# peterpengwei/bwa-mem-quickassist

Hardware: AMD Instinct MI355X
Metric: aligned reads/sec (150 bp PE vs hg38) at 1/2/4/8 MI355X; SAM bit-exact vs CPU (higher is better)
Workload: dtype int16; 1 GPU; pe10m -- BASELINE.json configs[2]: 10000000 x 2 x 150bp read pairs per GPU per step through the whole DP path (fused seed extension with the right extension started from the device's left score, ksw_global2 + traceback, mate-rescue ksw_align2), task generator in place of the hg38 index (SURVEY.md §8d), streamed in 2 chunks, inputs resident in HBM; seeding, chaining and SAM text are host stages out; pairs_per_gpu=10000000, reads_per_gpu=20000000, chunks=2, seeded_reads_per_gpu=19999921, global_tasks_per_gpu=17000000, rescue_tasks_per_gpu=600000, rescue_batches=1, streams=3, parallelism=static shard x1, one process per GPU, no collective on the data path

## Files before the change

### bwa-mem-quickassist_amd/__init__.py

```python
import ctypes as C
import os

import numpy as np

_HERE = os.path.dirname(os.path.abspath(__file__))
LIB_PATH = os.path.join(_HERE, "libbwamem_hip.so")
DROPIN_PATH = os.path.join(_HERE, "libbwamem_hip_dropin.so")
HEADER_PATH = os.path.join(os.path.dirname(_HERE), "include", "bwamem_hip.h")

BMH_OK, BMH_E_NODEVICE, BMH_E_HIP, BMH_E_ARG, BMH_E_RANGE, BMH_E_NOMEM, BMH_E_CIGAR_CAP = 0, -1, -2, -3, -4, -5, -6
BMH_F_QREV, BMH_F_TREV, BMH_F_TPAC, BMH_F_QCOMP = 1, 2, 4, 8

EXT_TASK = np.dtype([("q_off", "<u8"), ("t_off", "<u8"), ("qlen", "<u2"), ("tlen", "<u2"),
                     ("h0", "<i4"), ("w", "<i2"), ("end_bonus", "<i2"), ("flags", "<u2"),
                     ("rsv", "<u2")])
EXT_RES = np.dtype([("score", "<i4"), ("qle", "<i4"), ("tle", "<i4"), ("gtle", "<i4"),
                    ("gscore", "<i4"), ("max_off", "<i4")])
SEED_TASK = np.dtype([("q_off", "<u8"), ("t_off", "<u8"), ("l_query", "<i4"), ("qbeg", "<i4"), ("len", "<i4"),
                      ("rbeg", "<i4"), ("wlen", "<i4"), ("flags", "<u2"), ("rsv", "<u2")])
SEED_RES = np.dtype([("qb", "<i4"), ("qe", "<i4"), ("rb", "<i4"), ("re", "<i4"), ("score", "<i4"), ("truesc", "<i4"),
                     ("w", "<i4"), ("n_ext", "<i4")])
GLB_TASK = np.dtype([("q_off", "<u8"), ("t_off", "<u8"), ("qlen", "<u2"), ("tlen", "<u2"),
                     ("w", "<i4"), ("cigar_off", "<u4"), ("cigar_cap", "<u4")])
GLB_RES = np.dtype([("score", "<i4"), ("n_cigar", "<i4")])
# ... 84 lines not shown
    _fields_ = [("l_seq", C.c_int32), ("name", C.c_char_p), ("comment", C.c_char_p), ("seq", C.c_void_p), ("qual", C.c_char_p), ("sam", C.c_void_p)]


class _RefAnn(C.Structure):
    _fields_ = [("offset", C.c_int64), ("len", C.c_int32), ("n_ambs", C.c_int32), ("gi", C.c_uint32), ("name", C.c_char_p), ("anno", C.c_char_p)]


class _RefIdx(C.Structure):
    _fields_ = [("l_pac", C.c_int64), ("n_seqs", C.c_int32), ("seed", C.c_uint32), ("anns", C.POINTER(_RefAnn))]


def make_refidx(contigs, l_pac=None, names=None):
    anns = (_RefAnn * max(len(contigs), 1))()
    for i, (off, ln) in enumerate(contigs):
        anns[i] = _RefAnn(int(off), int(ln), 0, 0, names[i] if names is not None else b"seq%d" % i, b"")
    idx = _RefIdx(int(l_pac if l_pac is not None else contigs[-1][0] + contigs[-1][1]), len(contigs), 11, anns)
    idx._keep = anns
    return idx


class _ChainStats(C.Structure):
    _fields_ = [("reads", C.c_int64), ("chains_in", C.c_int64), ("chains_out", C.c_int64), ("seeds", C.c_int64), ("equal_keys", C.c_int64),
                ("kernel_ms", C.c_float)]


CHAIN_OPT = np.dtype([("w", "<i4"), ("max_chain_gap", "<i4"), ("min_seed_len", "<i4"), ("max_occ", "<i4"), ("split_len", "<i4"),
                      ("split_width", "<i4"), ("mask_level", "<f4"), ("chain_drop_ratio", "<f4")])


def _take_chains(out, n):
    res = []
    for k in range(n):
        chains = []
        for ci in range(out[k].n):
            c = out[k].a[ci]
            sd = np.zeros(c.n, dtype=SEED)
            if c.n:
                C.memmove(sd.ctypes.data, c.seeds, c.n * SEED.itemsize)
            chains.append(sd)
            _libc.free(c.seeds)
        if out[k].a:
            _libc.free(C.cast(out[k].a, C.c_void_p))
        res.append(chains)
    return res


class _DriverStats(C.Structure):
    _fields_ = [(n, C.c_int64) for n in ("rounds", "ext_tasks", "seeds_extended", "seeds_skipped", "pool_bytes", "seeds_speculated", "short_sw")]


_lib = None


def lib():
    global _lib
    if _lib is None:
        if not os.path.exists(LIB_PATH):
            raise BmhError(BMH_E_NODEVICE, f"{LIB_PATH} not built; run __graft_entry__.build()")
        L = C.CDLL(LIB_PATH)
        L.bmh_strerror.restype = C.c_char_p
        L.bmh_last_error.restype = C.c_char_p
        L.bmh_last_error.argtypes = [C.c_void_p]
        for name in ("bmh_ctx_destroy", "bmh_ctx_sync"):
            getattr(L, name).argtypes = [C.c_void_p]
        L.bmh_ctx_create.argtypes = [C.POINTER(C.c_void_p), C.c_int]
        L.bmh_ctx_set_params.argtypes = [C.c_void_p, C.c_void_p]
        L.bmh_ctx_set_stream.argtypes = [C.c_void_p, C.c_void_p]
        L.bmh_ctx_set_qcap.argtypes = [C.c_void_p, C.c_int]
        L.bmh_ctx_set_wide_extension.argtypes = [C.c_void_p, C.c_int]
        L.bmh_extend_wide_stats.argtypes = [C.c_void_p, C.POINTER(C.c_int64), C.POINTER(C.c_float)]
        L.bmh_global_long_stats.argtypes = [C.c_void_p, C.POINTER(C.c_int64), C.POINTER(C.c_float)]
        L.bmh_ctx_set_wide_sw.argtypes = [C.c_void_p, C.c_int]
        L.bmh_sw_wide_stats.argtypes = [C.c_void_p, C.POINTER(C.c_int64), C.POINTER(C.c_float)]
        L.bmh_ctx_reserve_staging.argtypes = [C.c_void_p, C.c_size_t, C.c_size_t]
        L.bmh_ctx_reserve_device.argtypes = [C.c_void_p, C.c_size_t, C.c_int64, C.c_size_t]
        L.bmh_ctx_reserve_kernels.argtypes = [C.c_void_p, C.c_int, C.c_int, C.c_int64, C.c_int]
        L.bmh_ctx_set_pac.argtypes = [C.c_void_p, C.c_void_p, C.c_int64]
        L.bmh_set_kernel_timing.argtypes = [C.c_void_p, C.c_int]
        L.bmh_last_kernel_ms.argtypes = [C.c_void_p, C.POINTER(C.c_float)]
        L.bmh_last_extend_bin_ms.argtypes = [C.c_void_p, C.POINTER(C.c_float)]
        L.bmh_last_global_bin_ms.argtypes = [C.c_void_p, C.POINTER(C.c_float)]
        L.bmh_last_global_bands.argtypes = [C.c_void_p, C.c_void_p, C.c_int64]
        L.bmh_last_global_bin_counts.argtypes = [C.c_void_p, C.c_void_p]
        L.bmh_ctx_set_extend_rows.argtypes = [C.c_void_p, C.c_int64]
        L.bmh_last_extend_rows.argtypes = [C.c_void_p, C.c_void_p, C.c_int64]
        L.bmh_last_extend_bands.argtypes = [C.c_void_p, C.c_void_p, C.c_int64]
        L.bmh_last_seedext_round_ms.argtypes = [C.c_void_p, C.POINTER(C.c_float)]
        L.bmh_extend_bin_ms_sum.argtypes = [C.c_void_p, C.POINTER(C.c_double), C.POINTER(C.c_longlong), C.c_int]
        L.bmh_upload_pool.argtypes = [C.c_void_p, C.c_void_p, C.c_size_t]
        L.bmh_extend_batch.argtypes = [C.c_void_p, C.c_void_p, C.c_size_t, C.c_void_p, C.c_int64, C.c_void_p]
        L.bmh_extend_batch_device.argtypes = [C.c_void_p, C.c_void_p, C.c_void_p, C.c_int64, C.c_void_p, C.c_void_p]
        L.bmh_seedext_batch.argtypes = [C.c_void_p, C.c_void_p, C.c_size_t, C.c_void_p, C.c_int64, C.c_void_p]
        L.bmh_seedext_batch_device.argtypes = [C.c_void_p, C.c_void_p, C.c_void_p, C.c_int64, C.c_void_p]
        L.bmh_seedext_submit.argtypes = [C.c_void_p, C.c_void_p, C.c_int64]
        L.bmh_seedext_wait.argtypes = [C.c_void_p, C.c_void_p]
        L.bmh_seedext_stats.argtypes = [C.c_void_p, C.c_void_p]
        L.bmh_ctx_set_bwt.argtypes = [C.c_void_p, C.c_void_p]
        L.bmh_smem_batch.argtypes = [C.c_void_p, C.c_void_p, C.c_int, C.c_void_p, C.c_void_p, C.c_void_p, C.c_size_t, C.c_void_p,
                                     C.c_void_p, C.c_size_t]
        L.bmh_sa_batch.argtypes = [C.c_void_p, C.c_void_p, C.c_int64, C.c_void_p]
        L.bmh_chain_batch.argtypes = [C.c_void_p, C.c_void_p, C.c_int64, C.c_int, C.c_void_p, C.c_void_p, C.c_void_p, C.c_void_p,
                                      C.c_void_p, C.c_void_p, C.c_void_p, C.c_uint64, C.c_void_p]
        L.bmh_seed_chain_batch.argtypes = [C.c_void_p, C.c_void_p, C.c_void_p, C.c_int64, C.c_int, C.c_void_p, C.c_void_p]
        L.bmh_chain_stats.argtypes = [C.c_void_p, C.c_void_p]
        L.bmh_matesw_batch.argtypes = [C.c_void_p, C.c_int64, C.c_void_p, C.c_int, C.c_void_p, C.c_void_p, C.c_void_p,
                                       C.c_void_p, C.c_void_p, C.c_void_p, C.c_void_p]
        L.bmh_matesw_device.argtypes = [C.c_void_p, C.c_int64, C.c_int, C.c_void_p, C.c_void_p, C.c_void_p, C.c_void_p, C.c_float,
                                        C.c_void_p]
        L.bmh_sw_batch.argtypes = [C.c_void_p, C.c_void_p, C.c_size_t, C.c_void_p, C.c_int64, C.c_void_p]
        L.bmh_sw_batch_device.argtypes = [C.c_void_p, C.c_void_p, C.c_void_p, C.c_int64, C.c_void_p]
        L.bmh_extend_batch_sharded.argtypes = [C.POINTER(C.c_void_p), C.c_int, C.c_void_p, C.c_size_t, C.c_void_p,
                                               C.c_int64, C.c_void_p]
        L.bmh_global_batch.argtypes = [C.c_void_p, C.c_void_p, C.c_size_t, C.c_void_p, C.c_int64, C.c_void_p,
                                       C.c_void_p, C.c_size_t]
        L.bmh_global_batch_device.argtypes = [C.c_void_p, C.c_void_p, C.c_void_p, C.c_int64, C.c_void_p, C.c_void_p,
                                              C.c_void_p]
        L.bmh_chain2aln_batch.argtypes = [C.c_void_p, C.c_int64, C.c_void_p, C.c_int, C.c_void_p, C.c_void_p,
                                          C.c_void_p, C.c_void_p, C.c_void_p]
        L.bmh_driver_stats.argtypes = [C.c_void_p, C.c_void_p]
        L.bmh_chains2regs_batch.argtypes = [C.c_void_p, C.c_int64, C.c_void_p, C.c_int, C.c_void_p, C.c_void_p, C.c_int, C.c_void_p]
        L.bmh_chains2regs_device.argtypes = [C.c_void_p, C.c_int64, C.c_int, C.c_void_p, C.c_void_p, C.c_int, C.c_void_p]
        L.bmh_seed_chain_regs_batch.argtypes = [C.c_void_p, C.c_void_p, C.c_void_p, C.c_int64, C.c_int, C.c_void_p, C.c_int, C.c_void_p]
        L.bmh_sort_dedup_batch.argtypes = [C.c_void_p, C.c_int, C.c_void_p, C.c_float]
        L.bmh_ctx_set_regs_dedup.argtypes = [C.c_void_p, C.c_int, C.c_float]
        L.bmh_last_dedup_stats.argtypes = [C.c_void_p, C.POINTER(C.c_int64), C.POINTER(C.c_int64), C.POINTER(C.c_float)]
        L.bmh_pestat_candidates.argtypes = [C.c_void_p, C.c_int64, C.c_int, C.c_void_p, C.c_void_p]
        L.bmh_pestat_from_candidates.argtypes = [C.c_void_p, C.c_int64, C.c_void_p, C.c_void_p, C.c_int]
        L.bmh_pestat_device.argtypes = [C.c_void_p, C.c_void_p, C.c_int64, C.c_int, C.c_void_p, C.c_void_p]
        L.bmh_ctx_set_regs_drop_exact.argtypes = [C.c_void_p, C.c_int]
        L.bmh_ctx_set_pestat_collect.argtypes = [C.c_void_p, C.c_int, C.c_void_p]
        L.bmh_last_pestat_candidates.argtypes = [C.c_void_p, C.c_void_p, C.c_int64, C.POINTER(C.c_float)]
        L.bmh_last_drop_exact_stats.argtypes = [C.c_void_p, C.POINTER(C.c_int64)]
        L.bmh_decide_batch.argtypes = [C.c_void_p, C.c_int64, C.c_void_p, C.c_int64, C.c_int] + [C.c_void_p] * 6
        L.bmh_decide_device.argtypes = [C.c_void_p] + L.bmh_decide_batch.argtypes
        L.bmh_ctx_set_decide_device.argtypes = [C.c_void_p, C.c_int]
        L.bmh_last_decide_stats.argtypes = [C.c_void_p, C.POINTER(C.c_int64), C.POINTER(C.c_int64), C.POINTER(C.c_float)]
        L.bmh_wanted_cigar_batch.argtypes = [C.c_void_p, C.c_void_p, C.c_void_p, C.c_int, C.c_int] + [C.c_void_p] * 7 + [C.c_size_t, C.c_void_p, C.c_size_t]
        L.bmh_wanted_cigar_device.argtypes = L.bmh_wanted_cigar_batch.argtypes
        L.bmh_ctx_set_refidx.argtypes = [C.c_void_p, C.c_void_p]
        L.bmh_ctx_set_wanted_device.argtypes = [C.c_void_p, C.c_int]
        L.bmh_phase2_device.argtypes = ([C.c_void_p] * 5 + [C.c_int64, C.c_int] + [C.c_void_p] * 8 + [C.c_int64, C.c_void_p, C.c_void_p, C.c_size_t,
                                        C.c_void_p, C.c_size_t])
        L.bmh_ctx_set_phase2_device.argtypes = [C.c_void_p, C.c_int]
        L.bmh_last_phase2_stats.argtypes = [C.c_void_p, C.c_void_p]
        L.bmh_sam_text_batch.argtypes = [C.c_void_p, C.c_void_p, C.c_void_p, C.c_int] + [C.c_void_p] * 10 + [C.c_char_p, C.c_void_p, C.c_void_p]
        L.bmh_sam_text_device.argtypes = [C.c_void_p] + L.bmh_sam_text_batch.argtypes
        L.bmh_ctx_set_refnames.argtypes = [C.c_void_p, C.c_void_p]
        L.bmh_ctx_set_samtext_device.argtypes = [C.c_void_p, C.c_int]
        L.bmh_last_samtext_stats.argtypes = [C.c_void_p, C.c_void_p]
        L.bmh_phase2_text_device.argtypes = [C.c_void_p] * 5 + [C.c_int64, C.c_int, C.c_void_p, C.c_void_p, C.c_char_p, C.c_void_p, C.c_void_p]
        L.bmh_ctx_set_phase2_text_device.argtypes = [C.c_void_p, C.c_int]
        L.bmh_last_phase2_text_stats.argtypes = [C.c_void_p, C.c_void_p]
        L.bmh_reads_sam_device.argtypes = [C.c_void_p, C.c_void_p, C.c_void_p, C.c_int, C.c_void_p, C.c_void_p, C.c_void_p, C.c_int64, C.c_int,
                                           C.c_void_p, C.c_char_p, C.c_void_p, C.c_void_p]
        L.bmh_last_reads_sam_stats.argtypes = [C.c_void_p, C.c_void_p]
        L.bmh_last_wanted_stats.argtypes = [C.c_void_p, C.POINTER(C.c_int64), C.POINTER(C.c_int64), C.POINTER(C.c_int64), C.POINTER(C.c_float)]
        L.bmh_region_cigar_batch.argtypes = [C.c_void_p, C.c_void_p, C.c_size_t, C.c_size_t, C.c_void_p, C.c_int64, C.c_void_p, C.c_int64,
                                             C.c_size_t, C.c_int, C.c_int, C.c_void_p, C.c_void_p, C.c_void_p]
        L.bmh_region_cigar_batch.restype = C.c_int
        L.bmh_region_cigar_batch_long.argtypes = L.bmh_region_cigar_batch.argtypes + [C.POINTER(C.c_void_p), C.POINTER(C.c_int64),
                                                                                      C.POINTER(C.c_void_p), C.POINTER(C.c_void_p)]
        L.bmh_region_cigar_batch_long.restype = C.c_int
        L.bmh_last_region_long_stats.argtypes = [C.c_void_p, C.POINTER(C.c_int64), C.POINTER(C.c_int64), C.POINTER(C.c_int64), C.POINTER(C.c_float)]
        L.bmh_ctx_set_region_long.argtypes = [C.c_void_p, C.c_int]
        L.bmh_last_reg2cigar_stats.argtypes = [C.c_void_p, C.POINTER(C.c_int64), C.POINTER(C.c_int64), C.POINTER(C.c_int64)]
        L.bmh_reg2cigar_batch.argtypes = [C.c_void_p, C.c_int64, C.c_void_p, C.c_void_p, C.c_int64, C.c_void_p, C.c_void_p,
# ... 49 lines not shown
        self._check(lib().bmh_ctx_set_stream(self._h, C.c_void_p(hip_stream_ptr)))

    def set_pac(self, pac, l_pac):
        pac = np.ascontiguousarray(pac, dtype=np.uint8)
        self._pac = pac
        self._check(lib().bmh_ctx_set_pac(self._h, _ptr(pac), int(l_pac)))
        return pac

    def set_qcap(self, q):
        self._check(lib().bmh_ctx_set_qcap(self._h, int(q)))

    def set_wide_extension(self, on=True):
        self._check(lib().bmh_ctx_set_wide_extension(self._h, 1 if on else 0))

    def extend_wide_stats(self):
        n, ms = C.c_int64(0), C.c_float(-1)
        self._check(lib().bmh_extend_wide_stats(self._h, C.byref(n), C.byref(ms)))
        return int(n.value), float(ms.value)

    def global_long_stats(self):
        n, ms = C.c_int64(0), C.c_float(-1)
        self._check(lib().bmh_global_long_stats(self._h, C.byref(n), C.byref(ms)))
        return int(n.value), float(ms.value)

    def set_wide_sw(self, on=True):
        self._check(lib().bmh_ctx_set_wide_sw(self._h, 1 if on else 0))

    def sw_wide_stats(self):
        n, ms = C.c_int64(0), C.c_float(-1)
        self._check(lib().bmh_sw_wide_stats(self._h, C.byref(n), C.byref(ms)))
        return int(n.value), float(ms.value)

    def reserve_staging(self, upload_bytes, download_bytes):
        self._check(lib().bmh_ctx_reserve_staging(self._h, int(upload_bytes), int(download_bytes)))

    def reserve_device(self, pool_bytes, max_tasks, cigar_words):
        self._check(lib().bmh_ctx_reserve_device(self._h, int(pool_bytes), int(max_tasks), int(cigar_words)))

    def reserve_kernels(self, seed_reads, seed_read_len, global_tasks, global_rows):
        self._check(lib().bmh_ctx_reserve_kernels(self._h, int(seed_reads), int(seed_read_len), int(global_tasks), int(global_rows)))

    def sync(self):
        self._check(lib().bmh_ctx_sync(self._h))

    def set_kernel_timing(self, on=True):
        self._check(lib().bmh_set_kernel_timing(self._h, 1 if on else 0))

    def last_kernel_ms(self):
        ms = C.c_float(-1)
        self._check(lib().bmh_last_kernel_ms(self._h, C.byref(ms)))
        return ms.value

    def last_extend_bin_ms(self):
        ms = (C.c_float * 6)()
        self._check(lib().bmh_last_extend_bin_ms(self._h, ms))
        return [float(x) for x in ms]

    def extend_bin_ms_sum(self, reset=True):
        ms = (C.c_double * 6)()
        n = C.c_longlong(0)
        self._check(lib().bmh_extend_bin_ms_sum(self._h, ms, C.byref(n), 1 if reset else 0))
        return [float(x) for x in ms], int(n.value)

    def last_seedext_round_ms(self):
        ms = (C.c_float * 4)()
        self._check(lib().bmh_last_seedext_round_ms(self._h, ms))
        return [float(x) for x in ms]

    def last_global_bin_ms(self):
        ms = (C.c_float * 3)()
        self._check(lib().bmh_last_global_bin_ms(self._h, ms))
        return [float(x) for x in ms]

    def last_global_bands(self, n):
        bands = np.zeros(int(n), dtype=np.uint8)
        self._check(lib().bmh_last_global_bands(self._h, _ptr(bands), int(n)))
        return bands

    def last_global_bin_counts(self):
        counts = np.zeros(8, dtype=np.uint32)
        self._check(lib().bmh_last_global_bin_counts(self._h, _ptr(counts)))
        return counts

    def set_extend_rows(self, cap):
        self._check(lib().bmh_ctx_set_extend_rows(self._h, int(cap)))

    def last_extend_rows(self, n):
        rows = np.zeros(int(n), dtype=np.uint16)
        self._check(lib().bmh_last_extend_rows(self._h, _ptr(rows), int(n)))
        return rows

    def last_extend_bands(self, n):
        bands = np.zeros(int(n), dtype=np.uint8)
        self._check(lib().bmh_last_extend_bands(self._h, _ptr(bands), int(n)))
        return bands

    def upload_pool(self, pool):
        pool = np.ascontiguousarray(pool, dtype=np.uint8)
        self._check(lib().bmh_upload_pool(self._h, _ptr(pool), pool.nbytes))

    def extend_batch(self, pool, tasks):
        pool = None if pool is None else np.ascontiguousarray(pool, dtype=np.uint8)
        tasks = np.ascontiguousarray(tasks, dtype=EXT_TASK)
        res = np.zeros(len(tasks), dtype=EXT_RES)
        self._check(lib().bmh_extend_batch(self._h, _ptr(pool), _nbytes(pool), _ptr(tasks), len(tasks), _ptr(res)))
        return res

    def seedext_batch(self, pool, tasks):
        pool = None if pool is None else np.ascontiguousarray(pool, dtype=np.uint8)
        tasks = np.ascontiguousarray(tasks, dtype=SEED_TASK)
        res = np.zeros(len(tasks), dtype=SEED_RES)
        self._check(lib().bmh_seedext_batch(self._h, _ptr(pool), _nbytes(pool), _ptr(tasks), len(tasks), _ptr(res)))
        return res

    def seedext_submit(self, tasks):
        tasks = np.ascontiguousarray(tasks, dtype=SEED_TASK)
        self._check(lib().bmh_seedext_submit(self._h, _ptr(tasks), len(tasks)))
        self._seed_pending = len(tasks)

    def seedext_wait(self):
        n, self._seed_pending = getattr(self, "_seed_pending", None) or 0, None
        res = np.zeros(n, dtype=SEED_RES)
        self._check(lib().bmh_seedext_wait(self._h, _ptr(res) if n else None))
        return res

    def seedext_batch_device(self, d_pool, d_tasks, n, d_res):
        self._check(lib().bmh_seedext_batch_device(self._h, C.c_void_p(d_pool), C.c_void_p(d_tasks), int(n), C.c_void_p(d_res)))

    def seedext_stats(self):
        st = (C.c_int64 * 5)()
        self._check(lib().bmh_seedext_stats(self._h, st))
        return dict(zip(("seeds", "left_tasks", "left_retries", "right_tasks", "right_retries"), [int(x) for x in st]))

    def global_batch(self, pool, tasks, cigar_words):
        pool = None if pool is None else np.ascontiguousarray(pool, dtype=np.uint8)
        tasks = np.ascontiguousarray(tasks, dtype=GLB_TASK)
        res = np.zeros(len(tasks), dtype=GLB_RES)
        cig = np.zeros(max(int(cigar_words), 1), dtype=np.uint32)
        self._check(lib().bmh_global_batch(self._h, _ptr(pool), _nbytes(pool), _ptr(tasks), len(tasks), _ptr(res),
                                           _ptr(cig), int(cigar_words)))
        return res, cig

    def region_cigar_batch(self, readpool, opool_bytes, reqs, tasks, task_cigar_words, cig_cap=24, md_cap=64):
        readpool = np.ascontiguousarray(readpool, dtype=np.uint8)
        reqs = np.ascontiguousarray(reqs, dtype=REGION_REQ)
        tasks = np.ascontiguousarray(tasks, dtype=GLB_TASK)
        res = np.zeros(len(reqs), dtype=REGION_RES)
        cig = np.zeros((max(len(reqs), 1), cig_cap), dtype=np.uint32)
        md = np.zeros((max(len(reqs), 1), md_cap), dtype=np.uint8)
        self._check(lib().bmh_region_cigar_batch(self._h, _ptr(readpool), readpool.nbytes, int(opool_bytes), _ptr(reqs), len(reqs),
                                                 _ptr(tasks), len(tasks), int(task_cigar_words), int(cig_cap), int(md_cap), _ptr(res),
                                                 _ptr(cig), _ptr(md)))
        return res, cig, md

    def region_cigar_batch_long(self, readpool, opool_bytes, reqs, tasks, task_cigar_words, cig_cap=24, md_cap=64, guard=0):
        readpool = np.ascontiguousarray(readpool, dtype=np.uint8)
        reqs = np.ascontiguousarray(reqs, dtype=REGION_REQ)
        tasks = np.ascontiguousarray(tasks, dtype=GLB_TASK)
        n = len(reqs)
        res_b = np.full(n * REGION_RES.itemsize + guard + 1, 0x5A, dtype=np.uint8)
        cig_b = np.full(max(n, 1) * cig_cap * 4 + guard, 0x5A, dtype=np.uint8)
        md_b = np.full(max(n, 1) * md_cap + guard, 0x5A, dtype=np.uint8)
        longs, n_long, lcig, lmd = C.c_void_p(), C.c_int64(-1), C.c_void_p(), C.c_void_p()
        self._check(lib().bmh_region_cigar_batch_long(self._h, _ptr(readpool), readpool.nbytes, int(opool_bytes), _ptr(reqs), n, _ptr(tasks),
                                                      len(tasks), int(task_cigar_words), int(cig_cap), int(md_cap), _ptr(res_b), _ptr(cig_b),
                                                      _ptr(md_b), C.byref(longs), C.byref(n_long), C.byref(lcig), C.byref(lmd)))
# ... 728 lines not shown
```

### bwa-mem-quickassist_amd/csrc/api.hip

```cpp
#include <algorithm>
#include <cstdio>
#include <cstdlib>
#include <cstring>
#include <functional>
#include <mutex>
#include <new>
#include <numeric>
#include <optional>
#include <vector>

#include "bmh_ctx.h"
#include "decide.h"
#include "wanted.h"
#include "samtext.h"
#include "../host/handoff_core.h"
#include "../host/pestat_core.h"

namespace bmh {

bmh_gate_fn g_gate_enter = nullptr, g_gate_leave = nullptr;
int g_wait_blocking = 0;

int set_hip_error(bmh_ctx *ctx, hipError_t e, const char *what)
{
// ... 178 lines not shown
	case BMH_E_HIP: return "HIP runtime error";
	case BMH_E_ARG: return "invalid argument";
	case BMH_E_RANGE: return "task outside the supported range";
	case BMH_E_NOMEM: return "out of memory";
	case BMH_E_CIGAR_CAP: return "CIGAR longer than the reserved slot range";
	default: return "unknown error";
	}
}

const char *bmh_last_error(const bmh_ctx_t *ctx) { return ctx ? ctx->last_error.c_str() : "null context"; }

int bmh_device_count(int *n)
{
	int c = 0;
	if (!n) return BMH_E_ARG;
	if (hipGetDeviceCount(&c) != hipSuccess) {
		*n = 0;
		return BMH_E_NODEVICE;
	}
	*n = c;
	return BMH_OK;
}

int bmh_ctx_create(bmh_ctx_t **out, int device)
{
	if (!out) return BMH_E_ARG;
	*out = nullptr;
	int c = 0;
	if (hipGetDeviceCount(&c) != hipSuccess || c <= 0) return BMH_E_NODEVICE;
	if (device < 0 || device >= c) return BMH_E_ARG;
	bmh_ctx *ctx = new (std::nothrow) bmh_ctx();
	if (!ctx) return BMH_E_NOMEM;
	ctx->device = device;
	hipError_t e;
	if ((e = hipSetDevice(device)) == hipSuccess && g_wait_blocking) {
		if (hipSetDeviceFlags(hipDeviceScheduleBlockingSync) != hipSuccess) (void)hipGetLastError();
	}
	if (e != hipSuccess || (e = hipStreamCreateWithFlags(&ctx->own_stream, hipStreamNonBlocking)) != hipSuccess ||
	    (e = hipMalloc((void **)&ctx->d_err, 16)) != hipSuccess || (e = hipMemset(ctx->d_err, 0, 16)) != hipSuccess ||
	    (e = hipHostMalloc((void **)&ctx->h_err, sizeof(int), hipHostMallocDefault)) != hipSuccess ||
	    (e = hipEventCreate(&ctx->ev0)) != hipSuccess || (e = hipEventCreate(&ctx->ev1)) != hipSuccess ||
	    (e = hipEventCreateWithFlags(&ctx->ev_fork, hipEventDisableTiming)) != hipSuccess ||
	    (e = hipEventCreateWithFlags(&ctx->ev_join, hipEventDisableTiming)) != hipSuccess ||
	    (e = hipEventCreateWithFlags(&ctx->ev_join2, hipEventDisableTiming)) != hipSuccess ||
	    (e = hipEventCreateWithFlags(&ctx->ev_wait, hipEventDisableTiming | hipEventBlockingSync)) != hipSuccess) {
		fprintf(stderr, "[bwamem_hip] context creation failed: %s\n", hipGetErrorString(e));
		bmh_ctx_destroy(ctx);
		return BMH_E_NODEVICE;
	}
	for (int b = 0; b <= kExtBinsMax; ++b)
		if (hipEventCreate(&ctx->ev_bin[b]) != hipSuccess || hipEventCreate(&ctx->ev_bin_end[b]) != hipSuccess) {
			bmh_ctx_destroy(ctx);
			return BMH_E_NODEVICE;
		}
	for (int b = 0; b < 5; ++b)
		if (hipEventCreate(&ctx->ev_sround[b]) != hipSuccess) {
			bmh_ctx_destroy(ctx);
			return BMH_E_NODEVICE;
		}
	for (int b = 0; b < 4; ++b)
		if (hipEventCreate(&ctx->ev_gbin[b]) != hipSuccess) {
			bmh_ctx_destroy(ctx);
			return BMH_E_NODEVICE;
		}
	ctx->stream = ctx->own_stream;
	(void)hipDeviceGetAttribute(&ctx->ncu, hipDeviceAttributeMultiprocessorCount, device);
	if (ctx->ncu <= 0) ctx->ncu = 256;
	if (const char *m = getenv("BMH_EXT_PERSIST")) ctx->ext_persist = atoi(m) != 0;
	if (const char *m = getenv("BMH_EXT_SPLIT96")) ctx->ext_split96 = atoi(m) != 0;
	if (const char *m = getenv("BMH_EXT_GRID_MULT")) ctx->ext_grid_mult = atoi(m) > 0 ? atoi(m) : ctx->ext_grid_mult;
	if (const char *m = getenv("BMH_EXT_STOP")) ctx->ext_stop = atoi(m) != 0;
	if (const char *m = getenv("BMH_EXT_NARROW")) ctx->ext_narrow = atoi(m) != 0;
	if (const char *m = getenv("BMH_EXT_BANDKEY")) ctx->ext_bandkey = atoi(m) != 0;
	if (const char *m = getenv("BMH_EXT_SMALL")) ctx->small_batch = atoi(m) >= 0 ? atoi(m) : ctx->small_batch;
	if (getenv("BMH_EXT_MODE")) ctx->ext_mode_forced = true;
	if (const char *m = getenv("BMH_EXT_MODE")) ctx->force_kernel = !strcmp(m, "lds") ? 1 : !strcmp(m, "reg") ? 2 : !strcmp(m, "grp") ? 3 : !strcmp(m, "lanex4") ? 4 : !strcmp(m, "wide") ? 5 : 0;
	if (const char *m = getenv("BMH_GLB_MODE")) ctx->glb_mode = !strcmp(m, "wave") ? 1 : 0;
	if (const char *m = getenv("BMH_SW_MODE")) ctx->sw_mode = !strcmp(m, "generic") ? 1 : 0;
	if (const char *m = getenv("BMH_SW_WAVE")) ctx->sw_wave = atoi(m) != 0;
	if (const char *m = getenv("BMH_GL_FAST")) ctx->glb_fast = atoi(m) != 0;
	if (const char *m = getenv("BMH_GLB_C32")) ctx->glb_c32 = atoi(m) != 0;
	if (const char *m = getenv("BMH_GLB_NARROW")) ctx->glb_narrow = atoi(m) != 0;
	if (const char *m = getenv("BMH_GLB_EXACT")) ctx->glb_exact = atoi(m) >= 7 ? 7 : atoi(m) >= 3 ? 3 : 0;
	if (const char *m = getenv("BMH_GRID_MULT")) ctx->grid_mult = atoi(m) > 0 ? atoi(m) : 1;
	if (const char *m = getenv("BMH_EXT_SCHED")) ctx->ext_sched = atoi(m) >= 0 && atoi(m) <= 4 ? atoi(m) : -1;
	*out = ctx;
	return BMH_OK;
}

static void pac_release(bmh_ctx_t *ctx);
void free_bwt_binding(void *p);

int bmh_ctx_destroy(bmh_ctx_t *ctx)
{
	if (!ctx) return BMH_OK;
	(void)hipSetDevice(ctx->device);
	if (ctx->stream) (void)stream_wait(ctx, ctx->stream);
	free_buf(ctx->d_pool), free_buf(ctx->d_tasks), free_buf(ctx->d_res), free_buf(ctx->d_order);
	free_buf(ctx->d_cigar), free_buf(ctx->d_scratch), free_buf(ctx->d_bins), free_buf(ctx->d_gband), free_buf(ctx->d_ext_rows), free_buf(ctx->d_eband), free_buf(ctx->d_zslab), free_buf(ctx->d_sw), free_buf(ctx->d_swrm);
	free_buf(ctx->d_seedws), free_buf(ctx->d_region), free_buf(ctx->d_chain), free_buf(ctx->d_wide_slab), free_buf(ctx->d_c2r);
	if (ctx->d_wide_stat) (void)hipFree(ctx->d_wide_stat);
	if (ctx->d_swl_stat) (void)hipFree(ctx->d_swl_stat);
	free_buf(ctx->d_swl), free_buf(ctx->d_dedup), free_buf(ctx->d_msw), free_buf(ctx->d_decide), free_buf(ctx->d_logk);
	free(ctx->h_logk);
	free_buf(ctx->d_refidx), free_buf(ctx->d_wanted);
	if (ctx->h_wstat) (void)hipHostFree(ctx->h_wstat);
	free_buf(ctx->d_refnames), free_buf(ctx->d_samtext), free_buf(ctx->d_sam_out);
	if (ctx->h_ststat) (void)hipHostFree(ctx->h_ststat);
	if (ctx->h_ptstat) (void)hipHostFree(ctx->h_ptstat);
	for (auto &e : ctx->ev_gather)
		if (e) (void)hipEventDestroy(e);
	for (auto &e : ctx->ev_samtext)
		if (e) (void)hipEventDestroy(e);
	for (auto &e : ctx->ev_wanted)
		if (e) (void)hipEventDestroy(e);
	for (auto &e : ctx->ev_decide)
		if (e) (void)hipEventDestroy(e);
	for (auto &e : ctx->ev_chain)
		if (e) (void)hipEventDestroy(e);
	for (auto &e : ctx->ev_dedup)
		if (e) (void)hipEventDestroy(e);
	free_buf(ctx->d_rlong), free_buf(ctx->d_lcig), free_buf(ctx->d_lmd);
	for (auto &e : ctx->ev_rlong)
		if (e) (void)hipEventDestroy(e);
	free_buf(ctx->d_pestat);
	for (auto &e : ctx->ev_pestat)
		if (e) (void)hipEventDestroy(e);
	for (auto &e : ctx->ev_plan)
		if (e) (void)hipEventDestroy(e);
	for (auto &h : ctx->hint) {
		if (h.ev) (void)hipEventDestroy(h.ev);
		if (h.h) (void)hipHostFree(h.h);
	}
	pac_release(ctx);
	if (ctx->bwt_bind) free_bwt_binding(ctx->bwt_bind);
	if (ctx->d_err) (void)hipFree(ctx->d_err);
	if (ctx->h_err) (void)hipHostFree(ctx->h_err);
	if (ctx->h_up.p) (void)hipHostFree(ctx->h_up.p);
	if (ctx->h_down.p) (void)hipHostFree(ctx->h_down.p);
	if (ctx->ev0) (void)hipEventDestroy(ctx->ev0);
	if (ctx->ev1) (void)hipEventDestroy(ctx->ev1);
	for (int b = 0; b <= kExtBinsMax; ++b)
	{
		if (ctx->ev_bin[b]) (void)hipEventDestroy(ctx->ev_bin[b]);
		if (ctx->ev_bin_end[b]) (void)hipEventDestroy(ctx->ev_bin_end[b]);
	}
	for (int b = 0; b < 4; ++b)
		if (ctx->ev_gbin[b]) (void)hipEventDestroy(ctx->ev_gbin[b]);
	for (int b = 0; b < 2; ++b)
		if (ctx->ev_glong[b]) (void)hipEventDestroy(ctx->ev_glong[b]);
	for (int b = 0; b < 2; ++b)
		if (ctx->ev_swl[b]) (void)hipEventDestroy(ctx->ev_swl[b]);
	for (int b = 0; b < 5; ++b)
		if (ctx->ev_sround[b]) (void)hipEventDestroy(ctx->ev_sround[b]);
	if (ctx->ev_fork) (void)hipEventDestroy(ctx->ev_fork);
	if (ctx->ev_join) (void)hipEventDestroy(ctx->ev_join);
	if (ctx->aux_stream) (void)hipStreamDestroy(ctx->aux_stream);
	if (ctx->ev_join2) (void)hipEventDestroy(ctx->ev_join2);
	if (ctx->ev_wait) (void)hipEventDestroy(ctx->ev_wait);
	if (ctx->aux2_stream) (void)hipStreamDestroy(ctx->aux2_stream);
	if (ctx->own_stream) (void)hipStreamDestroy(ctx->own_stream);
	delete ctx;
	return BMH_OK;
}

int bmh_ctx_set_params(bmh_ctx_t *ctx, const bmh_params_t *p)
{
	if (!ctx || !p) return BMH_E_ARG;
	if (p->e_del < 0 || p->e_ins < 0 || p->o_ins < 0 || p->o_del < 0) {
		ctx->last_error = "need e_del>=0, e_ins>=0, o_del>=0, o_ins>=0";
		return BMH_E_RANGE;
	}
	ctx->params = *p;
	DevParams &d = ctx->dev;
	d.o_del = p->o_del, d.e_del = p->e_del, d.o_ins = p->o_ins, d.e_ins = p->e_ins, d.zdrop = p->zdrop;
	d.max_mat = 0;
	int mn = 0;
	for (int i = 0; i < 25; ++i) d.max_mat = std::max(d.max_mat, (int)p->mat[i]), mn = std::min(mn, (int)p->mat[i]);
	d.bias = -mn;
	{
		int8_t lo = 127;
		for (int i = 0; i < 25; ++i) lo = std::min(lo, p->mat[i]);
// ... 150 lines not shown
int bmh_ctx_sync(bmh_ctx_t *ctx)
{
	if (!ctx) return BMH_E_ARG;
	BMH_HIP(ctx, hipSetDevice(ctx->device));
	BMH_HIP(ctx, stream_wait(ctx, ctx->stream));
	return fetch_err(ctx);
}

int bmh_set_kernel_timing(bmh_ctx_t *ctx, int enable)
{
	if (!ctx) return BMH_E_ARG;
	ctx->timing = enable != 0;
	ctx->ev_valid = false;
	return BMH_OK;
}

int bmh_last_kernel_ms(bmh_ctx_t *ctx, float *ms)
{
	if (!ctx || !ms) return BMH_E_ARG;
	*ms = -1.f;
	if (!ctx->ev_valid) return BMH_OK;
	BMH_HIP(ctx, hipEventSynchronize(ctx->ev1));
	BMH_HIP(ctx, hipEventElapsedTime(ms, ctx->ev0, ctx->ev1));
	return BMH_OK;
}

int bmh_last_extend_bin_ms(bmh_ctx_t *ctx, float ms[6])
{
	if (!ctx || !ms) return BMH_E_ARG;
	for (int b = 0; b < kExtBins; ++b) ms[b] = -1.f;
	if (!ctx->ev_bin_valid) return BMH_OK;
	BMH_HIP(ctx, hipEventSynchronize(ctx->ev1));
	for (int b = 0; b < kExtBins; ++b) BMH_HIP(ctx, hipEventElapsedTime(&ms[b], ctx->ev_bin[b], ctx->ev_bin_end[b]));
	return BMH_OK;
}

int bmh_extend_bin_ms_sum(bmh_ctx_t *ctx, double ms[6], long long *launches, int reset)
{
	if (!ctx || !ms) return BMH_E_ARG;
	for (int b = 0; b < kExtBins; ++b) ms[b] = ctx->ext_bin_ms_sum[b];
	if (launches) *launches = ctx->ext_bin_launches;
	if (reset) {
		for (int b = 0; b < kExtBins; ++b) ctx->ext_bin_ms_sum[b] = 0.0;
		ctx->ext_bin_launches = 0;
	}
	return BMH_OK;
}

int bmh_last_seedext_round_ms(bmh_ctx_t *ctx, float ms[4])
{
	if (!ctx || !ms) return BMH_E_ARG;
	ms[0] = ms[1] = ms[2] = ms[3] = -1.f;
	if (!ctx->ev_sround_valid) return BMH_OK;
	BMH_HIP(ctx, hipEventSynchronize(ctx->ev_sround[4]));
	for (int b = 0; b < 4; ++b) BMH_HIP(ctx, hipEventElapsedTime(&ms[b], ctx->ev_sround[b], ctx->ev_sround[b + 1]));
	return BMH_OK;
}

int bmh_last_global_bin_ms(bmh_ctx_t *ctx, float ms[3])
{
	if (!ctx || !ms) return BMH_E_ARG;
	ms[0] = ms[1] = ms[2] = -1.f;
	if (!ctx->ev_gbin_valid) return BMH_OK;
	BMH_HIP(ctx, hipEventSynchronize(ctx->ev_gbin[3]));
	for (int b = 0; b < 3; ++b) BMH_HIP(ctx, hipEventElapsedTime(&ms[b], ctx->ev_gbin[b], ctx->ev_gbin[b + 1]));
	return BMH_OK;
}

int bmh_last_global_bands(bmh_ctx_t *ctx, uint8_t *bands, int64_t n)
{
	if (!ctx || !bands || n <= 0 || n != ctx->gband_n || !ctx->d_gband.p) return BMH_E_ARG;
	BMH_HIP(ctx, hipSetDevice(ctx->device));
	BMH_HIP(ctx, stream_wait(ctx, ctx->stream));
	BMH_HIP(ctx, hipMemcpy(bands, ctx->d_gband.p, (size_t)n, hipMemcpyDeviceToHost));
	return BMH_OK;
}

int bmh_last_global_bin_counts(bmh_ctx_t *ctx, uint32_t counts[8])
{
	if (!ctx || !counts || !ctx->gbins_valid || !ctx->d_bins.p) return BMH_E_ARG;
	BMH_HIP(ctx, hipSetDevice(ctx->device));
	BMH_HIP(ctx, stream_wait(ctx, ctx->stream));
	BMH_HIP(ctx, hipMemcpy(counts, ctx->d_bins.p, kSortBins * sizeof(uint32_t), hipMemcpyDeviceToHost));
	return BMH_OK;
}

int bmh_ctx_set_extend_rows(bmh_ctx_t *ctx, int64_t cap)
{
	if (!ctx || cap < 0 || cap > 0xffffffffLL) return BMH_E_ARG;
	ctx->ext_rows_cap = cap, ctx->ext_rows_n = 0;
	return BMH_OK;
}

int bmh_last_extend_rows(bmh_ctx_t *ctx, uint16_t *rows, int64_t n)
{
	if (!ctx || !rows || n <= 0 || n > ctx->ext_rows_n || !ctx->d_ext_rows.p) return BMH_E_ARG;
	BMH_HIP(ctx, hipSetDevice(ctx->device));
	BMH_HIP(ctx, stream_wait(ctx, ctx->stream));
	BMH_HIP(ctx, hipMemcpy(rows, ctx->d_ext_rows.p, (size_t)n * sizeof(uint16_t), hipMemcpyDeviceToHost));
	return BMH_OK;
}

int bmh_last_extend_bands(bmh_ctx_t *ctx, uint8_t *bands, int64_t n)
{
	if (!ctx || !bands || n <= 0 || n != ctx->eband_n || !ctx->d_eband.p) return BMH_E_ARG;
	BMH_HIP(ctx, hipSetDevice(ctx->device));
	BMH_HIP(ctx, stream_wait(ctx, ctx->stream));
	BMH_HIP(ctx, hipMemcpy(bands, ctx->d_eband.p, (size_t)n, hipMemcpyDeviceToHost));
	return BMH_OK;
}


int bmh_extend_batch_device(bmh_ctx_t *ctx, const uint8_t *d_pool, const bmh_ext_task_t *d_tasks, int64_t n,
                            bmh_ext_result_t *d_res, const uint32_t *d_order)
{
	if (!ctx || n < 0 || (n > 0 && (!d_pool || !d_tasks || !d_res))) return BMH_E_ARG;
	if (!ctx->have_params) return BMH_E_ARG;
	if (n > 0xffffffffLL) return BMH_E_ARG;
	BMH_HIP(ctx, hipSetDevice(ctx->device));
	return launch_extend(ctx, d_pool, d_tasks, n, d_res, d_order, ctx->qcap);
}

static int validate_ext(bmh_ctx *ctx, const bmh_ext_task_t *t, int64_t n, size_t pool_bytes, int *qmax)
{
	int qm = 1;
	for (int64_t k = 0; k < n; ++k) {
		const bmh_ext_task_t &x = t[k];
		const bool qr = x.flags & BMH_F_QREV, tr = x.flags & BMH_F_TREV, tp = x.flags & BMH_F_TPAC;
		const uint64_t qlo = qr ? x.q_off - (x.qlen ? x.qlen - 1 : 0) : x.q_off, thi_len = x.tlen;
		const uint64_t tlo = tr ? x.t_off - (x.tlen ? x.tlen - 1 : 0) : x.t_off;
		const uint64_t tspace = tp ? (uint64_t)(ctx->dev.l_pac << 1) : (uint64_t)pool_bytes;
		if (tp && !ctx->dev.pac) {
			ctx->last_error = "task " + std::to_string(k) + " has BMH_F_TPAC but no reference was uploaded (bmh_ctx_set_pac)";
			return BMH_E_ARG;
		}
		if ((qr && x.qlen && x.q_off + 1 < x.qlen) || (tr && x.tlen && x.t_off + 1 < x.tlen) || qlo + x.qlen > pool_bytes ||
		    tlo + thi_len > tspace) {
			ctx->last_error = "task " + std::to_string(k) + " reads outside the sequence pool";
			return BMH_E_ARG;
		}
		const int h0 = x.h0 < 0 ? 0 : x.h0;
		if (!ctx->wide_ext && (int64_t)h0 + (int64_t)x.qlen * ctx->dev.max_mat > kScoreLimit) {
			ctx->last_error = "task " + std::to_string(k) + ": h0 + qlen*max(mat) exceeds the 16-bit score range";
			return BMH_E_RANGE;
		}
		if (ctx->wide_ext && (int64_t)h0 + (int64_t)x.qlen * ctx->dev.max_mat > kWideScoreLimit) {
			ctx->last_error = "task " + std::to_string(k) + ": h0 + qlen*max(mat) exceeds the wide extension's score range (2^24)";
			return BMH_E_RANGE;
		}
		qm = std::max(qm, (int)x.qlen);
	}
	*qmax = qm;
	return BMH_OK;
}

int bmh_extend_batch(bmh_ctx_t *ctx, const uint8_t *pool, size_t pool_bytes, const bmh_ext_task_t *tasks, int64_t n,
                     bmh_ext_result_t *results)
{
	if (!ctx || n < 0 || (n > 0 && (!tasks || !results))) return BMH_E_ARG;
	if (!ctx->have_params) return BMH_E_ARG;
	if (n == 0) return BMH_OK;
	if (n > 0xffffffffLL) return BMH_E_ARG;
	if (!pool && !ctx->pool_resident) return BMH_E_ARG;
	int qmax = 1, rc;
	if ((rc = validate_ext(ctx, tasks, n, pool ? pool_bytes : ctx->pool_bytes, &qmax))) return rc;
	GateGuard gate;
// ... 618 lines not shown
	if (n > 0 && (!pool || !tasks || !results)) return BMH_E_ARG;
	std::vector<int> qmax((size_t)std::max(n_ctx, 0));
	return run_sharded(
	    ctxs, n_ctx, n,
	    [&](bmh_ctx *c, size_t g, int64_t lo, int64_t m) { return m > 0x7fffffffLL ? BMH_E_ARG : validate_seeds(c, tasks + lo, m, pool_bytes, &qmax[g]); },
	    [&](Stager &st, size_t g, int64_t lo, int64_t m) {
		    return enqueue_batch(st, false, pool, pool_bytes, tasks + lo, m, results + lo, [&](bmh_ctx *c, auto p, auto t, auto r) {
			    return launch_seedext(c, p, t, m, r, qmax[g]);
		    });
	    });
}

int bmh_sw_batch_sharded(bmh_ctx_t *const *ctxs, int n_ctx, const uint8_t *pool, size_t pool_bytes, const bmh_sw_task_t *tasks, int64_t n,
                         bmh_sw_result_t *results)
{
	if (n > 0 && (!pool || !tasks || !results)) return BMH_E_ARG;
	struct SwShape {
		int qmax = 1, tmax = 1, qmin = 65535;
	};
	std::vector<SwShape> shape((size_t)std::max(n_ctx, 0));
	return run_sharded(
	    ctxs, n_ctx, n,
	    [&](bmh_ctx *c, size_t g, int64_t lo, int64_t m) {
		    SwShape &s = shape[g];
		    return validate_sw(c, tasks + lo, m, pool_bytes, &s.qmax, &s.tmax, &s.qmin);
	    },
	    [&](Stager &st, size_t g, int64_t lo, int64_t m) {
		    return enqueue_batch(st, false, pool, pool_bytes, tasks + lo, m, results + lo, [&](bmh_ctx *c, auto p, auto t, auto r) {
			    return launch_sw(c, p, t, m, r, shape[g].qmax, shape[g].tmax, shape[g].qmin);
		    });
	    });
}

int bmh_global_batch_sharded(bmh_ctx_t *const *ctxs, int n_ctx, const uint8_t *pool, size_t pool_bytes, const bmh_glb_task_t *tasks, int64_t n,
                             bmh_glb_result_t *results, uint32_t *cigar_pool, size_t cigar_words)
{
	if (n > 0 && (!pool || !tasks || !results)) return BMH_E_ARG;
	std::vector<std::vector<uint32_t>> back((size_t)std::max(n_ctx, 0));
	std::vector<GlbShape> shape((size_t)std::max(n_ctx, 0));
	const int rc = run_sharded(
	    ctxs, n_ctx, n,
	    [&](bmh_ctx *c, size_t g, int64_t lo, int64_t m) {
		    return m > 0xffffffffLL ? BMH_E_ARG : validate_glb(c, tasks + lo, m, pool_bytes, cigar_pool != nullptr, cigar_words, &shape[g]);
	    },
	    [&](Stager &st, size_t g, int64_t lo, int64_t m) {
		    const GlbShape &gs = shape[g];
		    back[g].resize(gs.cig_hi > gs.cig_lo ? gs.cig_hi - gs.cig_lo : 0);
		    const CigarDown cig{cigar_words, back[g].data(), gs.cig_lo, back[g].size()};
		    return enqueue_batch(
		        st, false, pool, pool_bytes, tasks + lo, m, results + lo,
		        [&](bmh_ctx *c, auto p, auto t, auto r) { return launch_global(c, p, t, m, r, (uint32_t *)c->d_cigar.p, nullptr, gs.qmax, gs.tmax, gs.wmax, gs.wraw, &gs.lg); },
		        &cig);
	    });
	if (rc && rc != BMH_E_CIGAR_CAP && rc != BMH_E_RANGE) return rc;
	for (int g = 0; g < n_ctx && n > 0; ++g) {
		const int64_t lo = n * g / n_ctx, hi = n * (g + 1) / n_ctx;
		if (back[(size_t)g].empty()) continue;
		for (int64_t k = lo; k < hi; ++k) {
			const bmh_glb_task_t &x = tasks[k];
			const size_t nw = std::min<size_t>((size_t)std::max(results[k].n_cigar, 0), x.cigar_cap);
			if (nw) memcpy(cigar_pool + x.cigar_off, back[(size_t)g].data() + ((size_t)x.cigar_off - shape[(size_t)g].cig_lo), nw * 4);
		}
	}
	return rc;
}

int bmh_ctx_reserve_staging(bmh_ctx_t *ctx, size_t upload_bytes, size_t download_bytes)
{
	if (!ctx) return BMH_E_ARG;
	int rc;
	BMH_HIP(ctx, hipSetDevice(ctx->device));
	if ((rc = ensure_host(ctx, ctx->h_up, upload_bytes)) || (rc = ensure_host(ctx, ctx->h_down, download_bytes))) return rc;
	return BMH_OK;
}

int bmh_ctx_reserve_device(bmh_ctx_t *ctx, size_t pool_bytes, int64_t max_tasks, size_t cigar_words)
{
	if (!ctx || max_tasks < 0) return BMH_E_ARG;
	int rc;
	const size_t N = (size_t)max_tasks;
	BMH_HIP(ctx, hipSetDevice(ctx->device));
	if (ctx->glb_narrow && (1 + (size_t)kSortBins) * N + 16 > ctx->d_gband.cap) ctx->gband_n = 0;
	if ((16 + (size_t)kSortBins * kSortKeysHost + (N + 1) / 2 + 1 + (size_t)kSortBins * N) * 4 > ctx->d_bins.cap) ctx->gbins_valid = false;
	if ((rc = ensure(ctx, ctx->d_pool, pool_bytes + 16)) || (rc = ensure(ctx, ctx->d_tasks, N * 40 + 64)) || (rc = ensure(ctx, ctx->d_res, N * 32 + 64)) ||
	    (rc = ensure(ctx, ctx->d_cigar, (cigar_words + 4) * 4)) ||
	    (rc = ensure(ctx, ctx->d_bins, (16 + (size_t)kSortBins * kSortKeysHost + (N + 1) / 2 + 1 + (size_t)kSortBins * N) * 4)) ||
	    (ctx->glb_narrow && (rc = ensure(ctx, ctx->d_gband, (1 + (size_t)kSortBins) * N + 16))))
		return rc;
	return BMH_OK;
}

int bmh_ctx_reserve_kernels(bmh_ctx_t *ctx, int seed_reads, int seed_read_len, int64_t global_tasks, int global_rows)
{
	if (!ctx || seed_reads < 0 || seed_read_len < 0 || global_tasks < 0 || global_rows < 0) return BMH_E_ARG;
	int rc;
	BMH_HIP(ctx, hipSetDevice(ctx->device));
	if (seed_reads > 0) {
		const size_t grid = std::min<size_t>(((size_t)seed_reads + 63) / 64, 1024 * 4);
		if ((rc = ensure(ctx, ctx->d_sw, grid * 3 * ((size_t)seed_read_len + 2) * 64 * 32))) return rc;
	}
	if (global_tasks > 0) {
		const size_t grid = std::min<size_t>(((size_t)global_tasks + 63) / 64, (size_t)std::max(ctx->ncu, 1) * 4 * 2);
		if ((rc = ensure(ctx, ctx->d_zslab, grid * (size_t)std::min(global_rows, 512) * 8 * 256))) return rc;
	}
	return BMH_OK;
}


int bmh_sort_dedup_batch(bmh_ctx_t *ctx, int n_reads, bmh_alnreg_v *regs, float mask_level_redun)
{
	if (!ctx || n_reads < 0 || (n_reads > 0 && !regs)) return BMH_E_ARG;
	size_t total = 0;
	for (int r = 0; r < n_reads; ++r) {
		if (regs[r].n && !regs[r].a) return BMH_E_ARG;
		if (regs[r].n > 0x7fffffffu - total) {
			ctx->last_error = "bmh_sort_dedup_batch: more than 2^31-1 regions in the batch";
			return BMH_E_ARG;
		}
		total += regs[r].n;
	}
	if (total == 0) {
		ctx->dedup_in = ctx->dedup_out = 0, ctx->dedup_ms = -1.f;
		return BMH_OK;
	}
	const size_t nr = (size_t)n_reads, o_off = 64, o_cnt = o_off + (nr + 1) * 8, o_reg = (o_cnt + nr * 8 + 63) & ~(size_t)63;
	const size_t b_reg = total * sizeof(bmh_alnreg_t), b_up = o_reg + b_reg, b_down = b_up - o_cnt;
	std::vector<uint8_t> up, down;
	try {
		up.resize(b_up), down.resize(b_down);
	} catch (const std::bad_alloc &) {
		ctx->last_error = "bmh_sort_dedup_batch: out of host memory";
		return BMH_E_NOMEM;
	}
	memset(up.data(), 0, o_off);
	unsigned long long *off = (unsigned long long *)(up.data() + o_off), *cnt = (unsigned long long *)(up.data() + o_cnt);
	size_t at = 0;
	for (int r = 0; r < n_reads; ++r) {
		off[r] = at, cnt[r] = regs[r].n;
		if (regs[r].n) memcpy(up.data() + o_reg + at * sizeof(bmh_alnreg_t), regs[r].a, regs[r].n * sizeof(bmh_alnreg_t));
		at += regs[r].n;
	}
	off[n_reads] = at;
	memset(up.data() + o_cnt + nr * 8, 0, o_reg - (o_cnt + nr * 8));
	GateGuard gate;
	BMH_HIP(ctx, hipSetDevice(ctx->device));
	Stager st(ctx);
	unsigned long long removed = 0;
	int rc = [&]() -> int {
		int e;
		if ((e = ensure(ctx, ctx->d_dedup, b_up)) || (e = st.stage(b_up, b_down + 64))) return e;
		uint8_t *d = (uint8_t *)ctx->d_dedup.p;
		if ((e = st.h2d(d, up.data(), b_up))) return e;
		if ((e = launch_region_dedup(ctx, (bmh_alnreg_t *)(d + o_reg), (const unsigned long long *)(d + o_off), (unsigned long long *)(d + o_cnt), n_reads,
		                             (unsigned long long)total, mask_level_redun, (unsigned long long *)d, ctx->d_err)))
			return e;
		if ((e = st.d2h(down.data(), d + o_cnt, b_down)) || (e = st.d2h(&removed, d, 8))) return e;
		return BMH_OK;
	}();
	if ((rc = st.end(rc))) return rc;
	const unsigned long long *kept = (const unsigned long long *)down.data();
	const uint8_t *ra = down.data() + (o_reg - o_cnt);
	for (int r = 0; r < n_reads; ++r) {
		if (regs[r].n <= 1) continue;
		if (kept[r] > regs[r].n) {
			ctx->last_error = "bmh_sort_dedup_batch: the device's counts are inconsistent";
			return BMH_E_ARG;
// ... 1622 lines not shown
```

### bwa-mem-quickassist_amd/csrc/bmh_ctx.h

```cpp
#pragma once
#include <hip/hip_runtime.h>
#include <stdint.h>
#include <string>
#include <vector>

#include "../../include/bwamem_hip.h"
#include "bmh_device.h"
#include "../host/regplan_core.h"

constexpr int kExtBinsMax = 6;

struct DevBuf {
	void *p = nullptr;
	size_t cap = 0;
};

struct bmh_ctx {
	int device = 0;
	hipStream_t own_stream = nullptr, stream = nullptr;
	bool have_params = false;
	bool glb_params = false;
	bmh_params_t params{};
	bmh::DevParams dev{};
	int qcap = 512;
	DevBuf d_pool, d_tasks, d_res, d_order, d_cigar, d_scratch;
	void *bwt_bind = nullptr;
	double smem_calls_per_base = 0.06, smem_intv_per_base = 0.35, smem_pos_per_base = 0.03;
	const uint8_t *h_pac = nullptr;
	DevBuf d_swrm;
	DevBuf d_sw;
	DevBuf d_zslab;
	int glb_mode = 0;
	int sw_mode = 0;
	int glb_fast = 1;
	int glb_narrow = 1;
	int glb_c32 = 1;
	int glb_exact = 7;
	bool gbins_valid = false;
	DevBuf d_gband;
	int64_t gband_n = 0;
	int sw_wave = 1;
	DevBuf d_bins;
	int grid_mult = 1;
	int ext_sched = -1;
	bool ext_mode_forced = false;
	int small_batch = 49152;
	int force_kernel = 0;
	bool pool_resident = false;
	size_t pool_bytes = 0;
	DevBuf h_up, h_down;
	int *d_err = nullptr;
	int *h_err = nullptr;
	bool timing = false;
	hipEvent_t ev0 = nullptr, ev1 = nullptr;
	bool ev_valid = false;
	hipEvent_t ev_bin[kExtBinsMax + 1] = {};
	hipEvent_t ev_bin_end[kExtBinsMax + 1] = {};
	hipStream_t aux_stream = nullptr;
	hipEvent_t ev_fork = nullptr, ev_join = nullptr;
	hipStream_t aux2_stream = nullptr;
	hipEvent_t ev_join2 = nullptr;
	hipEvent_t ev_wait = nullptr;
	bool ev_bin_valid = false;
	int ext_split96 = 1;
	double ext_bin_ms_sum[kExtBinsMax + 1] = {};
	long long ext_bin_launches = 0;
	hipEvent_t ev_gbin[4] = {};
	bool ev_gbin_valid = false;
	hipEvent_t ev_sround[5] = {};
	bool ev_sround_valid = false;
	std::string last_error;
	bmh_driver_stats_t dstats{};
	int ncu = 256;
	bool ext_persist = false;
	int ext_grid_mult = 2;
	int ext_stop = 1;
	int64_t ext_rows_cap = 0;
	DevBuf d_ext_rows;
	int64_t ext_rows_n = 0;
	int ext_narrow = 1;
	int ext_bandkey = 1;
	DevBuf d_eband;
	int64_t eband_n = 0;
	static constexpr int kHintKinds = 6;
	struct BinHint {
		uint32_t *h = nullptr;
		hipEvent_t ev = nullptr;
		bool pending = false, valid = false;
		uint32_t cnt[8] = {};
	} hint[kHintKinds];
	DevBuf d_seedws;
	DevBuf d_region;
	DevBuf d_rlong;
	DevBuf d_lcig, d_lmd;
	hipEvent_t ev_rlong[4] = {};
	long long rlong_regions = -1, rlong_words = -1, rlong_md = -1;
	float rlong_ms = -1.f;
	bool region_long = false;
	long long r2c_regions = -1, r2c_long_device = -1, r2c_redone_host = -1;
	bmh_seedext_stats_t sstats{};
	int64_t seed_pending_n = -1;
	DevBuf d_chain;
	hipEvent_t ev_chain[2] = {};
	bmh_chain_stats_t cstats{-1, -1, -1, -1, -1, -1.f};
	DevBuf d_c2r;
	bool wide_ext = false;
	bool wide_last = false;
	unsigned long long *d_wide_stat = nullptr;
	double wide_ms_sum = 0.0;
	long long wide_total = 0;
	DevBuf d_wide_slab;
	hipEvent_t ev_glong[2] = {};
	double glong_ms_sum = 0.0;
	bool wide_sw = false;
	unsigned long long *d_swl_stat = nullptr;
	DevBuf d_swl;
	hipEvent_t ev_swl[2] = {};
	double swl_ms_sum = 0.0;
	bool regs_dedup = false;
	float regs_dedup_mask = 0.95f;
// ... 61 lines not shown
	{
		if (leave) leave();
	}
	GateGuard(const GateGuard &) = delete;
	GateGuard &operator=(const GateGuard &) = delete;
};

int set_hip_error(bmh_ctx *ctx, hipError_t e, const char *what);

struct DevSeedTables {
	int n_reads;
	const int *len;
	const uint32_t *coff;
	const bmh_smem_call_t *calls;
	const uint64_t *ioff;
	const bmh_smem_intv_t *intv;
	const uint64_t *sa_off, *sa_pos;
	uint64_t n_calls, n_intv, n_pos;
	const uint8_t *pool;
	const uint64_t *read_off;
};
struct DevChains {
	int n_reads;
	const unsigned long long *coff, *soff;
	const uint32_t *cn;
	const bmh_seed_t *seeds;
	const uint32_t *n_keys;
	unsigned long long tc, ts;
	unsigned long long n_equal;
	float kernel_ms;
};
int chain_compact_device(bmh_ctx *ctx, const bmh_chain_opt_t *o, int64_t l_pac, const DevSeedTables &t, DevChains *out);
typedef int (*SeedTablesFn)(bmh_ctx *ctx, const DevSeedTables &t, void *user);
int seed_tables_device(bmh_ctx *ctx, const bmh_smem_opt_t *o, int max_occ, int n_reads, const bmh_read_t *reads, SeedTablesFn fn, void *user);
struct ResidentRegs {
	const unsigned long long *roff = nullptr;
	const bmh_alnreg_t *reg = nullptr;
	long long total = 0, kmax = 1, opool_cap = 0;
	bool neg = false;
};
int reads_regs_check(bmh_ctx *ctx, const bmh_smem_opt_t *so, const bmh_chain_opt_t *co, int64_t l_pac, int n_reads, const bmh_read_t *reads,
                     int min_seed_len, const char *who);
int reads_regs_resident(bmh_ctx *ctx, const bmh_smem_opt_t *so, const bmh_chain_opt_t *co, int64_t l_pac, int n_reads, const bmh_read_t *reads,
                        int min_seed_len, const bmh_sam_opt_t *o, ResidentRegs *out);
extern int g_wait_blocking;
inline hipError_t stream_wait(bmh_ctx *ctx, hipStream_t s)
{
	if (!g_wait_blocking || !ctx->ev_wait) return hipStreamSynchronize(s);
	const hipError_t e = hipEventRecord(ctx->ev_wait, s);
	return e != hipSuccess ? e : hipEventSynchronize(ctx->ev_wait);
}
int ensure(bmh_ctx *ctx, DevBuf &b, size_t bytes);
int ensure_host(bmh_ctx *ctx, DevBuf &b, size_t bytes);

#define BMH_HIP(ctx, call)                                                   \
	do {                                                                     \
		hipError_t e_ = (call);                                              \
		if (e_ != hipSuccess) return bmh::set_hip_error((ctx), e_, #call);   \
	} while (0)

constexpr long long kPersistentGrid = 256LL * 32 * 4;

inline bool ext_gaps_too_large(const bmh_params_t &p)
{
	return (long long)p.o_del + p.e_del > 65535 || (long long)p.o_ins + p.e_ins > 65535 || p.e_del > 16383 || p.e_ins > 16383;
}
int launch_extend(bmh_ctx *ctx, const uint8_t *d_pool, const bmh_ext_task_t *d_tasks, int64_t n,
                  bmh_ext_result_t *d_res, const uint32_t *d_order, int qmax, const uint32_t *d_n = nullptr, int kind = 0);
int launch_seedext(bmh_ctx *ctx, const uint8_t *d_pool, const bmh_seed_task_t *d_tasks, int64_t n,
                   bmh_seed_result_t *d_res, int qmax);
const uint32_t *seedext_counters(const bmh_ctx *ctx);
inline long long ext_resident_waves(const bmh_ctx *ctx, int waves_per_simd) { return (long long)ctx->ncu * 4 * waves_per_simd; }
constexpr int kLdsQcap = 13632;
constexpr int kWideLdsQcap = 12544;
int launch_extend_wide(bmh_ctx *ctx, const uint8_t *d_pool, const bmh_ext_task_t *d_tasks, int64_t n, bmh_ext_result_t *d_res,
                       const uint32_t *d_order, const uint32_t *d_count, int qmax, long long grid_cap = 0);
int wide_stats_begin(bmh_ctx *ctx);
int launch_extend_lds(bmh_ctx *ctx, const uint8_t *d_pool, const bmh_ext_task_t *d_tasks, int64_t n,
                      bmh_ext_result_t *d_res, const uint32_t *d_order, const uint32_t *d_count, int qmax, long long grid_cap = 0);
constexpr int kSortKeysHost = 2048;
int sort_tasks_begin(bmh_ctx *ctx, int64_t n, uint32_t **counts, uint32_t **lists);
int sort_tasks_finish(bmh_ctx *ctx, int64_t n, const uint32_t *d_order, unsigned blocks, const uint32_t *d_n = nullptr,
                      uint32_t *d_total = nullptr, const uint8_t *d_payload = nullptr, uint8_t *d_plists = nullptr);
int launch_global_lane(bmh_ctx *ctx, int c, const uint8_t *d_pool, const bmh_glb_task_t *d_tasks, int64_t n,
                       bmh_glb_result_t *d_res, uint32_t *d_cigar, const uint32_t *d_order, const uint32_t *d_count,
                       int rows_cap, const uint8_t *d_band = nullptr);
int launch_global_narrow(bmh_ctx *ctx, int wlo, const uint8_t *d_pool, const bmh_glb_task_t *d_tasks, int64_t n, bmh_glb_result_t *d_res,
                         uint32_t *d_cigar, const uint32_t *d_order, const uint32_t *d_count, int rows_cap, const uint8_t *d_band = nullptr);
constexpr int kExtBins = 6;
constexpr int kWideBin = 6;
constexpr int kSortBins = 8;
constexpr int kGrpTcapHost = 1024;

constexpr int kCapBin = 7;
constexpr int kSortBlocks = 512;
constexpr uint16_t kNoTask = 0xffff;
static_assert(kSortBins * kSortKeysHost <= kNoTask, "binkey is 16 bits wide and keeps one value for entries without a task");

__device__ __forceinline__ int ext_bin_of(int qlen, int tlen, int mode)
{
	if (mode == 1 || qlen < 1) return 5;
	if (mode == 3 && qlen <= 256 && tlen > kGrpTcapHost) return 3;
	return qlen <= 32 ? 0 : qlen <= 64 ? 1 : qlen <= 128 ? 2 : qlen <= 256 ? 3 : (qlen <= 512 && mode == 4) ? 4 : 5;
}

__device__ __forceinline__ bool ext_goes_wide(int qlen, int h0, int max_mat)
{
	return (long long)max(h0, 0) + (long long)qlen * max_mat > kScoreLimit || qlen > kLdsQcap;
}

__device__ __forceinline__ int ext_sort_key(int bin, int qlen, int tlen, int h0, int cls = -1)
{
	if (bin > 4) return 0;
	const int qlo = bin == 0 ? 1 : (16 << bin) + 1, qsh = bin < 2 ? 1 : bin;
	const int rows = min(tlen, 2 * qlen + 8) >> (bin > 2 ? bin - 2 : 0);
	return ((max(qlen - qlo, 0) >> qsh) * 8 + (cls >= 0 ? cls : min(max(h0, 0) >> 4, 7))) * 16 + min(rows >> 4, 15);
}

struct ExtBinRule {
	int mode;
	int wide;
	int max_mat, qmax;
	bmh_ext_result_t *out;
	int *err_flag;
};

__device__ __forceinline__ int ext_task_bin(const ExtBinRule &r, int qlen, int tlen, int h0)
{
	return qlen > r.qmax ? kCapBin : r.wide && (r.wide == 2 || ext_goes_wide(qlen, h0, r.max_mat)) ? kWideBin : ext_bin_of(qlen, tlen, r.mode);
}

__device__ __forceinline__ int ext_binkey_of(const ExtBinRule &r, int qlen, int tlen, int h0, size_t idx, int cls = -1)
{
	const int bin = ext_task_bin(r, qlen, tlen, h0);
	if (bin == kCapBin) {
		int *p = (int *)(r.out + idx);
		p[0] = INT32_MIN, p[1] = p[2] = p[3] = p[4] = p[5] = 0;
		atomicExch(r.err_flag, BMH_E_RANGE);
	}
	return bin * kSortKeysHost + ext_sort_key(bin, qlen, tlen, h0, cls);
}

struct ExtBinned {
	ExtBinRule rule;
	uint32_t *hist;
	uint16_t *binkey;
	unsigned blocks;
	uint8_t *band;
	bool tiny;
};
int extend_binned_begin(bmh_ctx *ctx, int64_t n, bmh_ext_result_t *d_res, int qmax, int kind, ExtBinned *p);
int extend_binned_finish(bmh_ctx *ctx, const uint8_t *d_pool, const bmh_ext_task_t *d_tasks, int64_t n, bmh_ext_result_t *d_res,
                         int qmax, int kind, const ExtBinned &p, uint32_t *d_total);

int launch_extend_grp(bmh_ctx *ctx, int nv, const uint8_t *d_pool, const bmh_ext_task_t *d_tasks, int64_t n,
                      bmh_ext_result_t *d_res, const uint32_t *d_order, const uint32_t *d_count);
int launch_extend_lanex(bmh_ctx *ctx, int lpt, const uint8_t *d_pool, const bmh_ext_task_t *d_tasks, int64_t n,
                        bmh_ext_result_t *d_res, const uint32_t *d_order, const uint32_t *d_count, int min_count);
int launch_sw(bmh_ctx *ctx, const uint8_t *d_pool, const bmh_sw_task_t *d_tasks, int64_t n, bmh_sw_result_t *d_res,
              int qcap, int tcap, int qmin);
inline bool sw_byte_gaps_wrap(const bmh_params_t &p) { return p.o_del + p.e_del > 255 || p.o_ins + p.e_ins > 255; }
int launch_sw_lane(bmh_ctx *ctx, int b, bool corr, bool word, const uint8_t *d_pool, const bmh_sw_task_t *d_tasks, int64_t n,
                   bmh_sw_result_t *d_res, const uint32_t *d_order, const uint32_t *d_count, uint16_t *d_rm, int rows_cap,
                   int grid, int pass2, uint32_t *d_next);
bool sw_wave_fits(int64_t n, int qcap, int tcap);
int launch_sw_wave(bmh_ctx *ctx, const uint8_t *d_pool, const bmh_sw_task_t *d_tasks, int64_t n, bmh_sw_result_t *d_res, int max_cols,
                   int tcap, const uint32_t *d_order = nullptr, const uint32_t *d_count = nullptr);
int launch_sw_generic(bmh_ctx *ctx, const uint8_t *d_pool, const bmh_sw_task_t *d_tasks, int64_t n,
                      bmh_sw_result_t *d_res, const uint32_t *d_order, const uint32_t *d_count, int qcap, int tcap, int wave_cols = 0,
// ... 71 lines not shown
```

### bwa-mem-quickassist_amd/csrc/bmh_device.h

```cpp
#pragma once
#include <hip/hip_runtime.h>
#include <stdint.h>

#include "../../include/bwamem_hip.h"

namespace bmh {

struct DevParams {
	int o_del, e_del, o_ins, e_ins, zdrop;
	int max_mat;
	int bias;
	int sw_shift;
	uint32_t matw[7];
	const uint8_t *pac;
	long long l_pac;
};

constexpr int kScoreLimit = 32000;
constexpr int kWideScoreLimit = 1 << 24;
constexpr int kNegInf16 = -16384;
constexpr int kGlbLaneWorst = 12000;

constexpr int DPP_ROW_SHR1 = 0x111, DPP_ROW_SHR2 = 0x112, DPP_ROW_SHR4 = 0x114, DPP_ROW_SHR8 = 0x118;
constexpr int DPP_WAVE_SHR1 = 0x138, DPP_ROW_BCAST15 = 0x142, DPP_ROW_BCAST31 = 0x143;

template <int CTRL, int ROW_MASK = 0xf>
__device__ __forceinline__ int dpp(int old, int src)
{
	return __builtin_amdgcn_update_dpp(old, src, CTRL, ROW_MASK, 0xf, false);
}

__device__ __forceinline__ int wave_scan_max(int v)
{
	constexpr int I = INT32_MIN;
	v = max(dpp<DPP_ROW_SHR1>(I, v), v);
	v = max(dpp<DPP_ROW_SHR2>(I, v), v);
	v = max(dpp<DPP_ROW_SHR4>(I, v), v);
	v = max(dpp<DPP_ROW_SHR8>(I, v), v);
	v = max(dpp<DPP_ROW_BCAST15, 0xa>(I, v), v);
	v = max(dpp<DPP_ROW_BCAST31, 0xc>(I, v), v);
	return v;
}

__device__ __forceinline__ int wave_reduce_max(int v)
{
	return __builtin_amdgcn_readlane(wave_scan_max(v), 63);
}

__device__ __forceinline__ int wave_shr1(int v, int lane0)
{
	return dpp<DPP_WAVE_SHR1>(lane0, v);
}

__device__ __forceinline__ int uni(int v) { return __builtin_amdgcn_readfirstlane(v); }

__device__ __forceinline__ int mat_at(const DevParams &P, int idx)
{
	return (int)(int8_t)(P.matw[idx >> 2] >> ((idx & 3) * 8));
}

__device__ __forceinline__ int seq_base(const uint8_t *pool, uint64_t off, int k, bool rev)
{
	return rev ? pool[off - (uint64_t)k] : pool[off + (uint64_t)k];
}

__device__ __forceinline__ int tgt_base(const uint8_t *pool, const DevParams &P, uint64_t off, int k, bool rev, bool tpac)
{
	if (!tpac) return seq_base(pool, off, k, rev);
	const long long p = rev ? (long long)off - k : (long long)off + k;
	const bool rs = p >= P.l_pac;
	const long long f = rs ? (P.l_pac << 1) - 1 - p : p;
	const int b = P.pac[f >> 2] >> ((~f & 3) << 1) & 3;
	return rs ? 3 - b : b;
}

#define BMH_OP16(name, text)                                                                                            \
	__device__ __forceinline__ int name(int a, int b)                                                                   \
	{                                                                                                                   \
		int d;                                                                                                          \
		asm(text " %0, %1, %2" : "=v"(d) : "v"(a), "v"(b));                                                             \
		return d;                                                                                                       \
	}
BMH_OP16(add16, "v_add_u16")
BMH_OP16(sub16, "v_sub_u16")
BMH_OP16(max16, "v_max_i16")
#undef BMH_OP16
__device__ __forceinline__ int maxu16(int a, int b)
{
	int d;
	asm("v_max_u16 %0, %1, %2" : "=v"(d) : "v"(a), "v"(b));
	return d;
}
__device__ __forceinline__ int subc16(int a, int k)
{
	int d;
	asm("v_sub_u16_e64 %0, %1, %2 clamp" : "=v"(d) : "v"(a), "s"(k));
	return d;
}
__device__ __forceinline__ int nonzero16(int a)
{
	int d;
	asm("v_min_u16 %0, 1, %1" : "=v"(d) : "v"(a));
	return d;
}
__device__ __forceinline__ int subk16(int a, int k)
{
	int d;
	asm("v_subrev_u16 %0, %1, %2" : "=v"(d) : "s"(k), "v"(a));
	return d;
}
template <int B> __device__ __forceinline__ int add_score(int sc4, int r)
{
	int d;
	if constexpr (B == 0) asm("v_add_u32_sdwa %0, sext(%1), %2 dst_sel:DWORD dst_unused:UNUSED_PAD src0_sel:BYTE_0 src1_sel:WORD_0" : "=v"(d) : "v"(sc4), "v"(r));
	if constexpr (B == 1) asm("v_add_u32_sdwa %0, sext(%1), %2 dst_sel:DWORD dst_unused:UNUSED_PAD src0_sel:BYTE_1 src1_sel:WORD_0" : "=v"(d) : "v"(sc4), "v"(r));
	if constexpr (B == 2) asm("v_add_u32_sdwa %0, sext(%1), %2 dst_sel:DWORD dst_unused:UNUSED_PAD src0_sel:BYTE_2 src1_sel:WORD_0" : "=v"(d) : "v"(sc4), "v"(r));
	if constexpr (B == 3) asm("v_add_u32_sdwa %0, sext(%1), %2 dst_sel:DWORD dst_unused:UNUSED_PAD src0_sel:BYTE_3 src1_sel:WORD_0" : "=v"(d) : "v"(sc4), "v"(r));
	return d;
}
__device__ __forceinline__ void max16_into_hi(int &r, int a, int b)
{
	asm("v_max_i16_sdwa %0, %1, %2 dst_sel:WORD_1 dst_unused:UNUSED_PRESERVE src0_sel:WORD_0 src1_sel:WORD_0" : "+v"(r) : "v"(a), "v"(b));
}

__device__ __forceinline__ void sub16_into_hi(int &r, int a, int b)
{
	asm("v_sub_u16_sdwa %0, %1, %2 dst_sel:WORD_1 dst_unused:UNUSED_PRESERVE src0_sel:WORD_0 src1_sel:WORD_0" : "+v"(r) : "v"(a), "v"(b));
}

__device__ __forceinline__ int band_cap(int qlen, int mx, int end_bonus, int o, int e)
{
	int x = qlen * mx + end_bonus - o;
	return x >= 0 ? x / e + 1 : 1;
}

}
```

### bwa-mem-quickassist_amd/csrc/global_kernel.hip

```cpp
#include "bmh_ctx.h"
#include "bmh_device.h"
#include "../host/glbband_core.h"
#include "../host/glbbin_core.h"

namespace bmh {

constexpr int kNegInf = -0x40000000;

struct CigarSink {
	uint32_t *base;
	int cap, nw, last_op, last_len;
	__device__ __forceinline__ void flush(int lane)
	{
		if (last_len > 0) {
			if (nw < cap && lane == 0) base[cap - 1 - nw] = (uint32_t)last_len << 4 | (uint32_t)last_op;
			++nw;
		}
	}
	__device__ __forceinline__ void push(int op, int len, int lane)
	{
		if (len <= 0) return;
		if (last_len > 0 && op == last_op) last_len += len;
		else {
			flush(lane);
// ... 187 lines not shown
				}
			}
			if (n_cigar > cigar_cap && lane == 0) atomicExch(err_flag, BMH_E_CIGAR_CAP);
		}
		if (lane == 0) out[idx].score = score, out[idx].n_cigar = n_cigar;
	}
}

__device__ __forceinline__ bool glb_lane_domain(const DevParams &P, int qlen, int tlen, int w, int lane_ok, int rows_cap)
{
	const int emax = max(P.e_del, P.e_ins), smax = max(P.bias, P.max_mat);
	const int worst = P.o_del + P.o_ins + emax * (qlen + tlen) + smax * max(qlen, tlen);
	return lane_ok && tlen <= rows_cap && worst < kGlbLaneWorst && P.o_del + P.o_ins < 4000 && w >= 0;
}

constexpr int kBandThreads = 256, kBandLanes = 8;
__global__ __launch_bounds__(kBandThreads) void glb_band_kernel(const uint8_t *__restrict__ pool, const bmh_glb_task_t *__restrict__ tasks,
                                                                const uint32_t *__restrict__ order, long long n, uint8_t *__restrict__ band,
                                                                DevParams P, int lane_ok, int rows_cap)
{
	__shared__ int8_t smat[32];
	if (threadIdx.x < 25) smat[threadIdx.x] = (int8_t)mat_at(P, threadIdx.x);
	__syncthreads();
	const int amax = bmh_glbband_amax(smat);
	const bool rule = bmh_glbband_applies(amax, P.o_del, P.e_del, P.o_ins, P.e_ins);
	const int g = threadIdx.x & (kBandLanes - 1);
	constexpr int kPer = kBandThreads / kBandLanes;
	for (long long k = (long long)blockIdx.x * kPer + threadIdx.x / kBandLanes; k < n; k += (long long)gridDim.x * kPer) {
		const uint32_t idx = order ? order[k] : (uint32_t)k;
		const uint4 *tp = (const uint4 *)(tasks + idx);
		const uint4 ta = tp[0], tb = tp[1];
		const int qlen = (int)(tb.x & 0xffff), tlen = (int)(tb.x >> 16);
		int w = (int)tb.y;
		if (rule && qlen >= 1 && tlen >= 1 && w >= abs(qlen - tlen) && glb_lane_domain(P, qlen, tlen, w, lane_ok, rows_cap)) {
			const bmh_gb_walk_t wk = bmh_glbband_walk(P.o_del, P.e_del, P.o_ins, P.e_ins, pool + ((uint64_t)ta.y << 32 | ta.x), qlen,
			                                          pool + ((uint64_t)ta.w << 32 | ta.z), tlen);
			const int per = ((wk.n + 8 * kBandLanes - 1) / (8 * kBandLanes)) * 8;
			const int from = min(g * per, wk.n), to = min(from + per, wk.n);
			const bmh_gb_part_t mine = bmh_glbband_part(smat, &wk, from, to);
			bmh_gb_part_t acc = {0, 0, 0};
#pragma unroll
			for (int j = 0; j < kBandLanes; ++j) {
				const bmh_gb_part_t nx = {__shfl(mine.s1, j, kBandLanes), __shfl(mine.d, j, kBandLanes), __shfl(mine.b, j, kBandLanes)};
				bmh_glbband_join(&acc, &nx);
			}
			w = bmh_glbband_from_lb(amax, P.o_del, P.e_del, P.o_ins, P.e_ins, qlen, tlen, w, acc.s1 + acc.b - wk.gap);
		}
		if (g == 0) band[k] = (uint8_t)(w < 0 || w > 255 ? 255 : w);
	}
}

__global__ __launch_bounds__(256) void glb_sort_hist_kernel(const bmh_glb_task_t *__restrict__ tasks,
                                                            const uint32_t *__restrict__ order, long long n,
                                                            uint32_t *__restrict__ hist, uint16_t *__restrict__ binkey,
                                                            DevParams P, int lane_ok, int rows_cap, int lds_qcap,
                                                            const uint8_t *__restrict__ band, int c32, int exact)
{
	__shared__ uint32_t lh[kSortBins * kSortKeysHost];
	for (int t = threadIdx.x; t < kSortBins * kSortKeysHost; t += 256) lh[t] = 0;
	__syncthreads();
	const long long chunk = (n + gridDim.x - 1) / gridDim.x, lo = chunk * blockIdx.x, hi = min(lo + chunk, n);
	for (long long k = lo + threadIdx.x; k < hi; k += 256) {
		const uint32_t idx = order ? order[k] : (uint32_t)k;
		const int qlen = tasks[idx].qlen, tlen = tasks[idx].tlen;
		int bin = 2, w = tasks[idx].w;
		if (glb_lane_domain(P, qlen, tlen, w, lane_ok, rows_cap)) {
			if (band) w = band[k];
			bin = bmh_glb_lane_bin(w, c32, exact);
		}
		if (bin == 2 && qlen > lds_qcap) bin = 4;
		const int bk = bin * kSortKeysHost + bmh_glb_sort_key(bin, tlen, w);
		binkey[k] = (uint16_t)bk;
		atomicAdd(&lh[bk], 1u);
	}
	__syncthreads();
	for (int t = threadIdx.x; t < kSortBins * kSortKeysHost; t += 256)
		if (lh[t]) atomicAdd(&hist[t], lh[t]);
}

int launch_global(bmh_ctx *ctx, const uint8_t *d_pool, const bmh_glb_task_t *d_tasks, int64_t n,
                  bmh_glb_result_t *d_res, uint32_t *d_cigar, const uint32_t *d_order, int qmax, int tmax,
                  int wmax, int wgate, const GlbLongShape *lg)
{
	ctx->gband_n = 0, ctx->gbins_valid = false;
	if (n <= 0) return BMH_OK;
	int rc;
	const size_t N = (size_t)n;
	const bool lane_ok = ctx->glb_mode == 0;
	const bool longb = lg && lg->qmax > 0;
	const int rows_cap = std::max(tmax, longb ? lg->tmax : 0) < 512 ? std::max(tmax, longb ? lg->tmax : 0) : 512;
	const long long budget = 8LL << 30;
	const int qcap = (std::min(qmax, kGlbLdsQcap) + 63) & ~63;
	const size_t state = glb_state_bytes(qcap);
	const long long ncol = qmax < 2LL * wmax + 1 ? qmax : 2LL * wmax + 1;
	long long zcap = ncol * (long long)tmax;
	zcap = (zcap + 15) & ~15LL;
	if (zcap < 16) zcap = 16;
	if (state > kGlbLdsBytes) return BMH_E_RANGE;
	const bool zlds = state + (size_t)zcap <= 64 * 1024;
	long long grid = n < (1LL << 20) ? n : (1LL << 20);
	if (lane_ok && grid > 8192) grid = 8192;
	if (!zlds) {
		long long g = budget / zcap;
		if (g < 1) return BMH_E_RANGE;
		if (g > 8192) g = 8192;
		if (grid > g) grid = g;
	}
	int ring = 64;
	long long zcap4 = 16, grid4 = 0;
	if (longb) {
		const int wq = std::min(lg->wmax, lg->qmax);
		while (ring < 2 * wq + 2 && ring < kGlbRingMax) ring <<= 1;
		zcap4 = (std::min<long long>(lg->qmax, 2LL * lg->wmax + 1) * (long long)lg->tmax + 15) & ~15LL;
		if (zcap4 < 16) zcap4 = 16;
		long long g = budget / zcap4;
		if (g < 1) return BMH_E_RANGE;
		grid4 = std::min<long long>({g, 8192, std::max<int64_t>(lg->n, 1)});
	}
	const size_t slab = std::max(zlds ? 0 : (size_t)grid * (size_t)zcap, longb ? (size_t)grid4 * (size_t)zcap4 : 0);
	if (slab && (rc = ensure(ctx, ctx->d_scratch, slab))) return rc;

	uint32_t *counts, *lists;
	if ((rc = sort_tasks_begin(ctx, n, &counts, &lists))) return rc;
	uint32_t *hist = counts + 16;
	uint16_t *binkey = (uint16_t *)(hist + (size_t)kSortBins * kSortKeysHost);
	long long cg = (n + 1023) / 1024;
	if (cg > 512) cg = 512;
	uint8_t *band = nullptr, *blists = nullptr;
	if (lane_ok && ctx->glb_narrow) {
		if ((rc = ensure(ctx, ctx->d_gband, (1 + (size_t)kSortBins) * N + 16))) return rc;
		band = (uint8_t *)ctx->d_gband.p, blists = band + ((N + 15) & ~(size_t)15);
		const long long bg = std::min<long long>((n * kBandLanes + kBandThreads - 1) / kBandThreads, (long long)ctx->ncu * 8 * 4);
		hipLaunchKernelGGL(glb_band_kernel, dim3((unsigned)bg), dim3(kBandThreads), 0, ctx->stream, d_pool, d_tasks, d_order, (long long)n,
		                   band, ctx->dev, 1, rows_cap);
		ctx->gband_n = n;
	}
	hipLaunchKernelGGL(glb_sort_hist_kernel, dim3((unsigned)cg), dim3(256), 0, ctx->stream, d_tasks, d_order, (long long)n, hist,
	                   binkey, ctx->dev, lane_ok ? 1 : 0, rows_cap, longb ? kGlbLdsQcap : 65535, band, ctx->glb_c32, ctx->glb_exact);
	if ((rc = sort_tasks_finish(ctx, n, d_order, (unsigned)cg, nullptr, nullptr, band, blists))) return rc;
	ctx->gbins_valid = true;
	const bool tm = ctx->timing;
	if (tm) BMH_HIP(ctx, hipEventRecord(ctx->ev0, ctx->stream));
	if (lane_ok) {
		if (tm) BMH_HIP(ctx, hipEventRecord(ctx->ev_gbin[0], ctx->stream));
		for (int b = 7; b >= 6; --b)
			if (ctx->glb_exact >= (b == 7 ? kGlbExactAll : kGlbExactLow) &&
			    (rc = launch_global_narrow(ctx, b == 7 ? 4 : 0, d_pool, d_tasks, n, d_res, d_cigar, lists + b * N, counts + b, rows_cap, blists ? blists + b * N : nullptr)))
				return rc;
		if (ctx->glb_c32 && (rc = launch_global_lane(ctx, 32, d_pool, d_tasks, n, d_res, d_cigar, lists + 5 * N, counts + 5, rows_cap,
		                                             blists ? blists + 5 * N : nullptr)))
			return rc;
		if ((rc = launch_global_lane(ctx, 64, d_pool, d_tasks, n, d_res, d_cigar, lists, counts + 0, rows_cap, blists))) return rc;
		if (tm) BMH_HIP(ctx, hipEventRecord(ctx->ev_gbin[1], ctx->stream));
		if (wgate > 31 && (rc = launch_global_lane(ctx, 96, d_pool, d_tasks, n, d_res, d_cigar, lists + 3 * N, counts + 3, rows_cap,
		                                             blists ? blists + 3 * N : nullptr)))
			return rc;
		if (wgate > 47 && (rc = launch_global_lane(ctx, 128, d_pool, d_tasks, n, d_res, d_cigar, lists + N, counts + 1, rows_cap,
		                                             blists ? blists + N : nullptr)))
			return rc;
	}
	if (tm) BMH_HIP(ctx, hipEventRecord(ctx->ev_gbin[2], ctx->stream));
	{
		const uint32_t *lst = lists + 2 * N, *cnt = counts + 2;
		if (zlds) {
			hipLaunchKernelGGL(global_kernel<true>, dim3((unsigned)grid), dim3(64), state + (size_t)zcap, ctx->stream, d_pool,
			                   d_tasks, lst, cnt, (long long)n, d_res, d_cigar, ctx->dev, qcap, zcap, (uint8_t *)nullptr, ctx->d_err);
		} else {
			hipLaunchKernelGGL(global_kernel<false>, dim3((unsigned)grid), dim3(64), state, ctx->stream, d_pool, d_tasks, lst, cnt,
			                   (long long)n, d_res, d_cigar, ctx->dev, qcap, zcap, (uint8_t *)ctx->d_scratch.p, ctx->d_err);
		}
		BMH_HIP(ctx, hipGetLastError());
	}
	if (tm) BMH_HIP(ctx, hipEventRecord(ctx->ev_gbin[3], ctx->stream));
	if (longb) {
		if (tm && !ctx->ev_glong[0]) {
			BMH_HIP(ctx, hipEventCreate(&ctx->ev_glong[0]));
			BMH_HIP(ctx, hipEventCreate(&ctx->ev_glong[1]));
		}
		if (tm) BMH_HIP(ctx, hipEventRecord(ctx->ev_glong[0], ctx->stream));
		hipLaunchKernelGGL((global_kernel<false, true>), dim3((unsigned)grid4), dim3(64), glb_ring_bytes(ring), ctx->stream, d_pool, d_tasks,
		                   lists + 4 * N, counts + 4, (long long)n, d_res, d_cigar, ctx->dev, ring, zcap4, (uint8_t *)ctx->d_scratch.p,
		                   ctx->d_err);
		BMH_HIP(ctx, hipGetLastError());
		if (tm) BMH_HIP(ctx, hipEventRecord(ctx->ev_glong[1], ctx->stream));
	}
	if (tm) {
		BMH_HIP(ctx, hipEventRecord(ctx->ev1, ctx->stream));
		ctx->ev_valid = true, ctx->ev_gbin_valid = lane_ok;
		if (longb) {
			float ms = 0.f;
			BMH_HIP(ctx, hipEventSynchronize(ctx->ev_glong[1]));
			BMH_HIP(ctx, hipEventElapsedTime(&ms, ctx->ev_glong[0], ctx->ev_glong[1]));
			ctx->glong_ms_sum += ms;
		}
	}
	return BMH_OK;
}

}
```

### bwa-mem-quickassist_amd/csrc/global_lane.hip

```cpp
#include <algorithm>
#include <cstdlib>
#include <type_traits>

#include "bmh_ctx.h"
#include "bmh_device.h"
#include "seq_stream.h"

namespace bmh {

constexpr int kNeg16 = -16384;
constexpr int kTbRows = 16;
constexpr int kStreamRows = 64;
constexpr int kStreamBatch = 2;
constexpr int kWindowBatch = 8;

__device__ __forceinline__ int sel3(int mask, int a, int b) { return __builtin_amdgcn_bitop3_b32(mask, a, b, 0xca); }

#ifndef BMH_GL_WAVES64
#define BMH_GL_WAVES64 3
#endif
#ifndef BMH_GL_WAVES32
#define BMH_GL_WAVES32 4
#endif
#ifndef BMH_GL_WAVES128
#define BMH_GL_WAVES128 2
#endif
#ifndef BMH_GL_WAVES96
#define BMH_GL_WAVES96 2
#endif


template <int C, bool FAST, bool SYM>
__global__ __launch_bounds__(64, (C <= 32 ? BMH_GL_WAVES32 : C <= 64 ? BMH_GL_WAVES64 : C <= 96 ? BMH_GL_WAVES96 : BMH_GL_WAVES128)) void global_lane_kernel(
    const uint8_t *__restrict__ pool, const bmh_glb_task_t *__restrict__ tasks, const uint32_t *__restrict__ order,
    const uint8_t *__restrict__ band, const uint32_t *__restrict__ count, long long n, bmh_glb_result_t *__restrict__ out,
    uint32_t *__restrict__ cigar_pool, DevParams P, uint32_t *__restrict__ zslab, int rows_cap, int *__restrict__ err_flag)
{
	constexpr int NW = (C + 31) / 32, NQ = C / 4, NB = C / 8;
	__shared__ uint2 srow[8];
	extern __shared__ __attribute__((aligned(16))) uint8_t dyn_lds[];
	const int lane = threadIdx.x;
	const int oe_del = P.o_del + P.e_del, oe_ins = P.o_ins + P.e_ins;
	const int e_del = P.e_del, e_ins = P.e_ins;
	if (lane < 5) {
		uint32_t lo = 0;
		for (int q = 0; q < 4; ++q) lo |= (uint32_t)(uint8_t)mat_at(P, lane * 5 + q) << (8 * q);
		srow[lane] = make_uint2(lo, (uint32_t)(uint8_t)mat_at(P, lane * 5 + 4));
	}
	const long long cnt = count ? (long long)*count : n;
	uint32_t *__restrict__ zbase = zslab + (size_t)blockIdx.x * (size_t)rows_cap * (size_t)(NB * 64);

	for (long long base = (long long)blockIdx.x * 64; base < cnt; base += (long long)gridDim.x * 64) {
		const bool valid = base + lane < cnt;
		const long long pos = cnt - 1 - (valid ? base + lane : base);
		const uint32_t idx = order ? order[pos] : (uint32_t)pos;
		const uint4 *tp = (const uint4 *)(tasks + idx);
		const uint4 ta = tp[0], tb = tp[1];
		const uint64_t q_off = (uint64_t)ta.y << 32 | ta.x;
		const int qlen = (int)(tb.x & 0xffff), tlen = (int)(tb.x >> 16);
		const int w = band ? (int)band[pos] : (int)tb.y;
		const bool want = (int)tb.w > 0;
		const bool bad = w < 0 || 2 * w + 2 > C || tlen > rows_cap;
		if (valid && bad) {
			out[idx].score = INT32_MIN, out[idx].n_cigar = 0;
			atomicExch(err_flag, BMH_E_RANGE);
		}
		const bool live = valid && !bad;

		int R[C + 1], QW[NQ];
#pragma unroll
		for (int s = 0; s <= C; ++s) {
			const int j = s - w;
			const int hd = j < 0 ? kNeg16 : (j == 0 ? 0 : (j <= w && j <= qlen ? -(P.o_ins + e_ins * j) : kNeg16));
			R[s] = (int)((uint32_t)kNeg16 << 16 | ((uint32_t)hd & 0xffffu));
		}
		uint8_t *strm = dyn_lds;
		uint32_t *qstage = (uint32_t *)dyn_lds;
#pragma unroll 1
		for (int v0 = 0; v0 < NQ; v0 += kWindowBatch) {
			uint32_t qw[kWindowBatch];
			seq_issue<kWindowBatch>(qw, pool, q_off, qlen, 4 * v0 - w, false, live);
			seq_finish<kWindowBatch>(qw, qlen, 4 * v0 - w, false, live);
#pragma unroll
			for (int v = 0; v < kWindowBatch; ++v) qstage[(v0 + v) * 64 + lane] = qw[v];
		}
#pragma unroll
		for (int v = 0; v < NQ; ++v) QW[v] = (int)qstage[v * 64 + lane];
		const int qsh = C - w;
		auto fill_stream = [&](int r0) {
			const uint4 tq = *(const uint4 *)(tasks + idx);
			const uint64_t q_off = (uint64_t)tq.y << 32 | tq.x, t_off = (uint64_t)tq.w << 32 | tq.z;
			int lane_now;
			asm volatile("v_mbcnt_lo_u32_b32 %0, -1, 0\n\tv_mbcnt_hi_u32_b32 %0, -1, %0" : "=v"(lane_now));
			glb_fill_stream<kStreamRows, kStreamBatch>(strm, lane_now, pool, t_off, tlen, q_off, qlen, r0, qsh, live);
		};
		int i = 0, score = kNeg16;
		for (; __builtin_amdgcn_ballot_w64(live && i < tlen) != 0; ++i) {
			const bool rowon = live && i < tlen;
			if ((i & (kStreamRows - 1)) == 0) fill_stream(i);
			int lane_now;
			asm volatile("v_mbcnt_lo_u32_b32 %0, -1, 0\n\tv_mbcnt_hi_u32_b32 %0, -1, %0" : "=v"(lane_now));
			const int sbyte = strm[(i & (kStreamRows - 1)) * 64 + lane_now];
			const int tcur = sbyte & 15, qin = sbyte >> 4;
			const uint2 row = srow[min(tcur, 4)];
			const int slo = rowon ? max(0, w - i) : C + 1;
			const int shi = rowon ? min(2 * w + 1, qlen - i + w) : C + 1;
			int am[NW];
#pragma unroll
			for (int v = 0; v < NW; ++v) {
				const int lo = min(max(slo - 32 * v, 0), 32), hi = min(max(shi - 32 * v, 0), 32);
				am[v] = hi > lo ? (int)((0xffffffffu >> (32 - (hi - lo))) << lo) : 0;
			}
			const int fill = i < w ? -(P.o_del + e_del * (i + 1)) : kNeg16;
			int f = kNeg16;
#pragma unroll
			for (int b = 0; b < NB; ++b) {
				if (__builtin_amdgcn_ballot_w64(slo <= 8 * b + 8 && shi > 8 * b) == 0) continue;
				const bool masked = !FAST || __builtin_amdgcn_ballot_w64(rowon && !(slo <= 8 * b && shi >= 8 * b + 8)) != 0;
				int dz12 = 0, dz34 = 0;
				auto cells = [&](auto MASKED) {
#pragma unroll
					for (int q4 = 0; q4 < 2; ++q4) {
						const int sc4 = (int)__builtin_amdgcn_perm(row.y, row.x, (unsigned)QW[2 * b + q4]);
#pragma unroll
						for (int c4 = 0; c4 < 4; ++c4) {
							const int s = 8 * b + 4 * q4 + c4;
							const int m = c4 == 0 ? add_score<0>(sc4, R[s]) : c4 == 1 ? add_score<1>(sc4, R[s]) : c4 == 2 ? add_score<2>(sc4, R[s]) : add_score<3>(sc4, R[s]);
							const int e = (int)((unsigned)R[s + 1] >> 16);
							const int h1 = max16(m, e);
							const int h = max16(h1, f);
							const int t1 = subk16(m, oe_del), e2 = subk16(e, e_del);
							const int t2 = SYM ? t1 : subk16(m, oe_ins), f2 = subk16(f, e_ins);
#ifdef BMH_GL_PERM_SIGNS
							const int x1 = sub16(m, e), x2 = sub16(h1, f), x3 = sub16(t1, e2), x4 = sub16(t2, f2);
							const int z12 = (int)__builtin_amdgcn_perm((unsigned)x1, (unsigned)x2, 0x0c0c0105u);
							const int z34 = (int)__builtin_amdgcn_perm((unsigned)x3, (unsigned)x4, 0x0c0c0105u);
							dz12 = __builtin_amdgcn_bitop3_b32((int)((unsigned)dz12 >> 1), z12, 0x8080, 0xf8);
							dz34 = __builtin_amdgcn_bitop3_b32((int)((unsigned)dz34 >> 1), z34, 0x8080, 0xf8);
#else
							int x12 = sub16(m, e), x34 = sub16(t1, e2);
							sub16_into_hi(x12, h1, f);
							sub16_into_hi(x34, t2, f2);
							dz12 = __builtin_amdgcn_bitop3_b32((int)((unsigned)dz12 >> 1), x12, (int)0x80008000u, 0xf8);
							dz34 = __builtin_amdgcn_bitop3_b32((int)((unsigned)dz34 >> 1), x34, (int)0x80008000u, 0xf8);
#endif
							if constexpr (decltype(MASKED)::value) {
								const int actv = (am[s / 32] << (31 - s % 32)) >> 31;
								f = sel3(actv, max16(f2, t2), kNeg16);
								R[s] = (int)__builtin_amdgcn_perm((unsigned)sel3(actv, max16(e2, t1), kNeg16), (unsigned)sel3(actv, h, fill), 0x05040100u);
							} else {
								f = max16(f2, t2);
								int r = h;
								max16_into_hi(r, e2, t1);
								R[s] = r;
							}
#ifdef BMH_GL_SCHED_CELL
							__builtin_amdgcn_sched_barrier(0);
#endif
						}
#ifdef BMH_GL_SCHED_Q4
						__builtin_amdgcn_sched_barrier(0);
#endif
					}
				};
				if (masked) cells(std::true_type{});
				else if constexpr (FAST) cells(std::false_type{});
#ifdef BMH_GL_PERM_SIGNS
				const uint32_t dz = (uint32_t)dz12 | (uint32_t)dz34 << 16;
#else
				const uint32_t dz = (uint32_t)dz12 >> 8 | (uint32_t)dz34;
#endif
				if (want) {
					const uint32_t *line = zbase + ((size_t)b * (size_t)rows_cap + (size_t)i) * 64;
					asm volatile("global_store_dword %0, %1, %2" : : "v"(lane * 4), "v"(dz), "s"(line) : "memory");
				}
			}
			if (__builtin_amdgcn_ballot_w64(live && i == tlen - 1)) {
				const int ss = qlen - tlen + w;
				int pick = 0;
#pragma unroll
				for (int c0 = 0; c0 < C; c0 += 32) {
					int T[16];
#pragma unroll
					for (int k = 0; k < 16; ++k) {
						const int a0 = c0 + 2 * k < C ? R[c0 + 2 * k] : 0, a1 = c0 + 2 * k + 1 < C ? R[c0 + 2 * k + 1] : 0;
						T[k] = (ss & 1) ? a1 : a0;
					}
#pragma unroll
					for (int bit = 1, len = 8; len >= 1; ++bit, len >>= 1)
#pragma unroll
						for (int k = 0; k < len; ++k) T[k] = (ss >> bit & 1) ? T[2 * k + 1] : T[2 * k];
					pick = (ss >> 5) == c0 / 32 ? T[0] : pick;
				}
				if (live && i == tlen - 1 && ss >= 0 && ss <= 2 * w) score = (int)(int16_t)(pick & 0xffff);
			}
#pragma unroll
			for (int v = 0; v + 1 < NQ; ++v) QW[v] = (int)__builtin_amdgcn_alignbyte((unsigned)QW[v + 1], (unsigned)QW[v], 1u);
			QW[NQ - 1] = (int)__builtin_amdgcn_alignbyte((unsigned)qin, (unsigned)QW[NQ - 1], 1u);
		}

		if (tlen == 0) score = qlen == 0 ? 0 : (qlen <= w ? -(P.o_ins + e_ins * qlen) : kNeg16);
		if (score <= -kGlbLaneWorst) score = -0x40000000;

		const uint2 tc = *(const uint2 *)((const uint8_t *)(tasks + idx) + 24);
		const uint32_t cigar_off = tc.x;
		const int cigar_cap = (int)tc.y;
		int n_cigar = 0;
		if (__builtin_amdgcn_ballot_w64(live && want)) {
			__builtin_amdgcn_fence(__ATOMIC_SEQ_CST, "workgroup");
			uint32_t *cg = cigar_pool + cigar_off;
			int ti = tlen - 1, tk = min(qlen, tlen - 1 + w + 1) - 1, which = 0, last_op = 0, last_len = 0, nw = 0;
			bool on = live && want;
			uint32_t *strip = (uint32_t *)dyn_lds;
			int cblk = -1, ctop = -1;
			while (__builtin_amdgcn_ballot_w64(on && ti >= 0 && tk >= 0)) {
				const bool act = on && ti >= 0 && tk >= 0;
				const int s = min(max(tk - (ti - w), 0), C - 1);
				if (__builtin_amdgcn_ballot_w64(act && ((s >> 3) != cblk || ti > ctop || ti <= ctop - kTbRows))) {
					if (act) {
						cblk = s >> 3, ctop = ti;
						const uint32_t *src = zbase + ((size_t)cblk * (size_t)rows_cap) * 64 + lane;
						uint32_t v[kTbRows];
#pragma unroll
						for (int k = 0; k < kTbRows; ++k) v[k] = ti - k >= 0 ? src[(size_t)(ti - k) * 64] : 0u;
#pragma unroll
						for (int k = 0; k < kTbRows; ++k) strip[k * 64 + lane] = v[k];
					}
				}
				if (act) {
					const uint32_t dzw = strip[(ctop - ti) * 64 + lane] >> (s & 7);
#ifdef BMH_GL_PERM_SIGNS
					which = which == 0 ? ((dzw >> 8 & 1) ? 2 : (int)(dzw & 1)) : which == 1 ? (int)(dzw >> 16 & 1) : (int)(dzw >> 23 & 2);
#else
					which = which == 0 ? ((dzw >> 16 & 1) ? 2 : (int)(dzw & 1)) : which == 1 ? (int)(dzw >> 8 & 1) : (int)(dzw >> 23 & 2);
#endif
					const int op = which == 0 ? 0 : (which == 1 ? 2 : 1);
					if (last_len > 0 && op == last_op) ++last_len;
					else {
						if (last_len > 0) {
							if (nw < cigar_cap) cg[cigar_cap - 1 - nw] = (uint32_t)last_len << 4 | (uint32_t)last_op;
							++nw;
						}
						last_op = op, last_len = 1;
					}
					ti -= which != 2;
					tk -= which != 1;
				}
			}
			if (on) {
				for (int pass = 0; pass < 2; ++pass) {
					const int op = pass == 0 ? 2 : 1, len = pass == 0 ? ti + 1 : tk + 1;
					if (len <= 0) continue;
					if (last_len > 0 && op == last_op) last_len += len;
					else {
						if (last_len > 0) {
							if (nw < cigar_cap) cg[cigar_cap - 1 - nw] = (uint32_t)last_len << 4 | (uint32_t)last_op;
							++nw;
						}
						last_op = op, last_len = len;
					}
				}
				if (last_len > 0) {
					if (nw < cigar_cap) cg[cigar_cap - 1 - nw] = (uint32_t)last_len << 4 | (uint32_t)last_op;
					++nw;
				}
				n_cigar = nw;
				const int shift = cigar_cap - nw;
				if (shift > 0 && nw <= cigar_cap) {
					__builtin_amdgcn_fence(__ATOMIC_SEQ_CST, "workgroup");
					for (int c = 0; c < nw; ++c) cg[c] = cg[shift + c];
				}
				if (nw > cigar_cap) atomicExch(err_flag, BMH_E_CIGAR_CAP);
			}
		}
		if (live) out[idx].score = score, out[idx].n_cigar = n_cigar;
	}
}

int launch_global_lane(bmh_ctx *ctx, int c, const uint8_t *d_pool, const bmh_glb_task_t *d_tasks, int64_t n,
                       bmh_glb_result_t *d_res, uint32_t *d_cigar, const uint32_t *d_order, const uint32_t *d_count,
                       int rows_cap, const uint8_t *d_band)
{
	if (n <= 0) return BMH_OK;
	int ncu = 256;
	(void)hipDeviceGetAttribute(&ncu, hipDeviceAttributeMultiprocessorCount, ctx->device);
	long long grid = (n + 63) / 64;
	const long long resident = (long long)ncu * 4 * (c <= 32 ? BMH_GL_WAVES32 : c <= 64 ? BMH_GL_WAVES64 : c <= 96 ? BMH_GL_WAVES96 : BMH_GL_WAVES128);
	if (grid > resident) grid = resident;
	const size_t slab = (size_t)grid * (size_t)rows_cap * (size_t)(c / 8) * 64 * 4;
	int rc = ensure(ctx, ctx->d_zslab, slab);
	if (rc) return rc;
	const bool fast = ctx->glb_fast != 0;
	const bool sym = ctx->dev.o_del + ctx->dev.e_del == ctx->dev.o_ins + ctx->dev.e_ins;
	const size_t lds = (size_t)std::max(c, kStreamRows) * 64;
#define BMH_LAUNCH_GL2(CC, FF, SS)                                                                                             \
	hipLaunchKernelGGL((global_lane_kernel<CC, FF, SS>), dim3((unsigned)grid), dim3(64), lds, ctx->stream, d_pool, d_tasks, d_order, \
	                   d_band, d_count, (long long)n, d_res, d_cigar, ctx->dev, (uint32_t *)ctx->d_zslab.p, rows_cap, ctx->d_err)
#define BMH_LAUNCH_GL(CC)                                                                                                      \
	do {                                                                                                                       \
		if (fast && sym) BMH_LAUNCH_GL2(CC, true, true);                                                                       \
		else if (fast) BMH_LAUNCH_GL2(CC, true, false);                                                                        \
		else if (sym) BMH_LAUNCH_GL2(CC, false, true);                                                                         \
		else BMH_LAUNCH_GL2(CC, false, false);                                                                                 \
	} while (0)
	if (c == 32) BMH_LAUNCH_GL(32);
	else if (c == 64) BMH_LAUNCH_GL(64);
	else if (c == 96) BMH_LAUNCH_GL(96);
	else if (c == 128) BMH_LAUNCH_GL(128);
	else return BMH_E_ARG;
#undef BMH_LAUNCH_GL
#undef BMH_LAUNCH_GL2
	BMH_HIP(ctx, hipGetLastError());
	return BMH_OK;
}

}
```

### bwa-mem-quickassist_amd/csrc/global_narrow.hip

```cpp
#include <algorithm>
#include <type_traits>

#include "bmh_ctx.h"
#include "bmh_device.h"
#include "seq_stream.h"

namespace bmh {

namespace {

constexpr int kNeg16 = -16384;
constexpr int kTbRows = 16;
constexpr int kStreamRows = 64;
constexpr int kStreamBatch = 2;
constexpr int kNarrowBlocks = 2;

__device__ __forceinline__ int sel3n(int mask, int a, int b) { return __builtin_amdgcn_bitop3_b32(mask, a, b, 0xca); }

__device__ __forceinline__ int lane_now()
{
	int l;
	asm volatile("v_mbcnt_lo_u32_b32 %0, -1, 0\n\tv_mbcnt_hi_u32_b32 %0, -1, %0" : "=v"(l));
	return l;
}
// ... 35 lines not shown

	int score = kNeg16;
	for (int i = 0; __builtin_amdgcn_ballot_w64(mine && i < tlen) != 0; ++i) {
		const bool rowon = mine && i < tlen;
		if ((i & (kStreamRows - 1)) == 0) fill_stream(i);
		const int lane = lane_now();
		const int sbyte = strm[(i & (kStreamRows - 1)) * 64 + lane];
		const int tcur = sbyte & 15, qin = sbyte >> 4;
		const uint2 row = srow[min(tcur, 4)];
		const bool masked = __builtin_amdgcn_ballot_w64(rowon && (i < W || i + W >= qlen)) != 0;
		uint32_t dzw[NB];
		auto cells = [&](auto MASKED) {
			int am = 0, fill = kNeg16;
			if constexpr (decltype(MASKED)::value) {
				const int lo = max(W - i, 0), hi = min(max(qlen - i + W, 0), NS);
				am = rowon && hi > lo ? (int)((0xffffffffu >> (32 - (hi - lo))) << lo) : 0;
				fill = i < W ? -(P.o_del + e_del * (i + 1)) : kNeg16;
			}
			int f = kNeg16, dz12 = 0, dz34 = 0, sc4 = 0;
#pragma unroll
			for (int s = 0; s < NS; ++s) {
				const int c4 = s & 3;
				if (c4 == 0) sc4 = (int)__builtin_amdgcn_perm(row.y, row.x, (unsigned)QW[s >> 2]);
				if ((s & 7) == 0) dz12 = dz34 = 0;
				const int m = c4 == 0 ? add_score<0>(sc4, R[s]) : c4 == 1 ? add_score<1>(sc4, R[s]) : c4 == 2 ? add_score<2>(sc4, R[s]) : add_score<3>(sc4, R[s]);
				const int e = s + 1 < NS ? (int)((unsigned)R[s + 1] >> 16) : (kNeg16 & 0xffff);
				const int h1 = max16(m, e);
				const int h = max16(h1, f);
				const int t1 = subk16(m, oe_del), e2 = subk16(e, e_del);
				const int t2 = SYM ? t1 : subk16(m, oe_ins), f2 = subk16(f, e_ins);
				int x12 = sub16(m, e), x34 = sub16(t1, e2);
				sub16_into_hi(x12, h1, f);
				sub16_into_hi(x34, t2, f2);
				dz12 = __builtin_amdgcn_bitop3_b32((int)((unsigned)dz12 >> 1), x12, (int)0x80008000u, 0xf8);
				dz34 = __builtin_amdgcn_bitop3_b32((int)((unsigned)dz34 >> 1), x34, (int)0x80008000u, 0xf8);
				if constexpr (decltype(MASKED)::value) {
					const int actv = (am << (31 - s)) >> 31;
					f = sel3n(actv, max16(f2, t2), kNeg16);
					R[s] = (int)__builtin_amdgcn_perm((unsigned)sel3n(actv, max16(e2, t1), kNeg16), (unsigned)sel3n(actv, h, fill), 0x05040100u);
				} else {
					f = max16(f2, t2);
					int r = h;
					max16_into_hi(r, e2, t1);
					R[s] = r;
				}
				if ((s & 7) == 7 || s == NS - 1) {
					const int n = (s & 7) + 1;
					dzw[s >> 3] = (uint32_t)dz12 >> (16 - n) | (uint32_t)dz34 >> (8 - n);
				}
			}
		};
		if (masked) cells(std::true_type{});
		else cells(std::false_type{});
		if (mine && want) {
#pragma unroll
			for (int b = 0; b < NB; ++b) {
				const uint32_t *line = zbase + ((size_t)b * (size_t)rows_cap + (size_t)i) * 64;
				asm volatile("global_store_dword %0, %1, %2" : : "v"(lane * 4), "v"(dzw[b]), "s"(line) : "memory");
			}
		}
		if (__builtin_amdgcn_ballot_w64(mine && i == tlen - 1)) {
			const int ss = qlen - tlen + W;
			int pick = kNeg16;
#pragma unroll
			for (int s = 0; s < NS; ++s) pick = ss == s ? R[s] : pick;
			if (mine && i == tlen - 1) score = (int)(int16_t)(pick & 0xffff);
		}
#pragma unroll
		for (int v = 0; v + 1 < NQ; ++v) QW[v] = (int)__builtin_amdgcn_alignbyte((unsigned)QW[v + 1], (unsigned)QW[v], 1u);
		QW[NQ - 1] = (int)__builtin_amdgcn_alignbyte((unsigned)qin, (unsigned)QW[NQ - 1], 1u);
	}
	return score;
}

}

#ifndef BMH_GN_WAVES_LO
#define BMH_GN_WAVES_LO 8
#endif
#ifndef BMH_GN_WAVES_HI
#define BMH_GN_WAVES_HI 6
#endif

template <int WLO, bool SYM>
__global__ __launch_bounds__(64, (WLO == 0 ? BMH_GN_WAVES_LO : BMH_GN_WAVES_HI)) void global_narrow_kernel(
    const uint8_t *__restrict__ pool, const bmh_glb_task_t *__restrict__ tasks, const uint32_t *__restrict__ order,
    const uint8_t *__restrict__ band, const uint32_t *__restrict__ count, long long n, bmh_glb_result_t *__restrict__ out,
    uint32_t *__restrict__ cigar_pool, DevParams P, uint32_t *__restrict__ zslab, int rows_cap, int *__restrict__ err_flag)
{
	__shared__ uint2 srow[8];
	__shared__ __attribute__((aligned(16))) uint8_t lds[kStreamRows * 64];
	static_assert(kStreamRows * 64 == kTbRows * 64 * 4, "one LDS area serves both");
	const int lane = threadIdx.x;
	if (lane < 5) {
		uint32_t lo = 0;
		for (int q = 0; q < 4; ++q) lo |= (uint32_t)(uint8_t)mat_at(P, lane * 5 + q) << (8 * q);
		srow[lane] = make_uint2(lo, (uint32_t)(uint8_t)mat_at(P, lane * 5 + 4));
	}
	const long long cnt = count ? (long long)*count : n;
	uint32_t *__restrict__ zbase = zslab + (size_t)blockIdx.x * (size_t)rows_cap * (size_t)(kNarrowBlocks * 64);

	for (long long base = (long long)blockIdx.x * 64; base < cnt; base += (long long)gridDim.x * 64) {
		const bool valid = base + lane < cnt;
		const long long pos = cnt - 1 - (valid ? base + lane : base);
		const uint32_t idx = order ? order[pos] : (uint32_t)pos;
		const uint4 tb = ((const uint4 *)(tasks + idx))[1];
		const int qlen = (int)(tb.x & 0xffff), tlen = (int)(tb.x >> 16);
		const int w = band ? (int)band[pos] : (int)tb.y;
		const bool want = (int)tb.w > 0;
		const bool bad = w < WLO || w > WLO + 3 || tlen > rows_cap;
		if (valid && bad) {
			out[idx].score = INT32_MIN, out[idx].n_cigar = 0;
			atomicExch(err_flag, BMH_E_RANGE);
		}
		const bool live = valid && !bad;

		int score = kNeg16;
		for (unsigned long long todo = __builtin_amdgcn_ballot_w64(live); todo != 0;) {
			const int wc = __builtin_amdgcn_readlane(w, (int)__builtin_ctzll(todo));
			const bool mine = live && w == wc;
			int sc = kNeg16;
#define BMH_GN_CASE(WW)                                                                                                \
	case WW:                                                                                                           \
		sc = narrow_rows<WW, SYM>(mine, want, qlen, tlen, idx, pool, tasks, P, srow, lds, zbase, rows_cap);            \
		break;
			switch (wc) {
				BMH_GN_CASE(WLO)
				BMH_GN_CASE(WLO + 1)
				BMH_GN_CASE(WLO + 2)
				BMH_GN_CASE(WLO + 3)
			}
#undef BMH_GN_CASE
			if (mine) score = sc;
			todo &= ~__builtin_amdgcn_ballot_w64(mine);
		}
		if (tlen == 0) score = qlen == 0 ? 0 : (qlen <= w ? -(P.o_ins + P.e_ins * qlen) : kNeg16);
		if (score <= -kGlbLaneWorst) score = -0x40000000;

		const uint2 tc = *(const uint2 *)((const uint8_t *)(tasks + idx) + 24);
		const uint32_t cigar_off = tc.x;
		const int cigar_cap = (int)tc.y;
		int n_cigar = 0;
		if (__builtin_amdgcn_ballot_w64(live && want)) {
			__builtin_amdgcn_fence(__ATOMIC_SEQ_CST, "workgroup");
			uint32_t *cg = cigar_pool + cigar_off;
			int ti = tlen - 1, tk = min(qlen, tlen - 1 + w + 1) - 1, which = 0, last_op = 0, last_len = 0, nw = 0;
			const bool on = live && want;
			uint32_t *strip = (uint32_t *)lds;
			int cblk = -1, ctop = -1;
			while (__builtin_amdgcn_ballot_w64(on && ti >= 0 && tk >= 0)) {
				const bool act = on && ti >= 0 && tk >= 0;
				const int s = min(max(tk - (ti - w), 0), 2 * w);
				if (__builtin_amdgcn_ballot_w64(act && ((s >> 3) != cblk || ti > ctop || ti <= ctop - kTbRows))) {
					if (act) {
						cblk = s >> 3, ctop = ti;
						const uint32_t *src = zbase + ((size_t)cblk * (size_t)rows_cap) * 64 + lane;
#pragma unroll 1
						for (int k0 = 0; k0 < kTbRows; k0 += kTbRows / 2) {
							uint32_t v[kTbRows / 2];
#pragma unroll
							for (int k = 0; k < kTbRows / 2; ++k) v[k] = ti - k0 - k >= 0 ? src[(size_t)(ti - k0 - k) * 64] : 0u;
#pragma unroll
							for (int k = 0; k < kTbRows / 2; ++k) strip[(k0 + k) * 64 + lane] = v[k];
						}
					}
				}
				if (act) {
					const uint32_t dzw = strip[(ctop - ti) * 64 + lane] >> (s & 7);
					which = which == 0 ? ((dzw >> 16 & 1) ? 2 : (int)(dzw & 1)) : which == 1 ? (int)(dzw >> 8 & 1) : (int)(dzw >> 23 & 2);
					const int op = which == 0 ? 0 : (which == 1 ? 2 : 1);
					if (last_len > 0 && op == last_op) ++last_len;
					else {
						if (last_len > 0) {
							if (nw < cigar_cap) cg[cigar_cap - 1 - nw] = (uint32_t)last_len << 4 | (uint32_t)last_op;
							++nw;
						}
						last_op = op, last_len = 1;
					}
					ti -= which != 2;
					tk -= which != 1;
				}
			}
			if (on) {
				for (int pass = 0; pass < 2; ++pass) {
					const int op = pass == 0 ? 2 : 1, len = pass == 0 ? ti + 1 : tk + 1;
					if (len <= 0) continue;
					if (last_len > 0 && op == last_op) last_len += len;
					else {
						if (last_len > 0) {
							if (nw < cigar_cap) cg[cigar_cap - 1 - nw] = (uint32_t)last_len << 4 | (uint32_t)last_op;
							++nw;
						}
						last_op = op, last_len = len;
					}
				}
				if (last_len > 0) {
					if (nw < cigar_cap) cg[cigar_cap - 1 - nw] = (uint32_t)last_len << 4 | (uint32_t)last_op;
					++nw;
				}
				n_cigar = nw;
				const int shift = cigar_cap - nw;
				if (shift > 0 && nw <= cigar_cap) {
					__builtin_amdgcn_fence(__ATOMIC_SEQ_CST, "workgroup");
					for (int c = 0; c < nw; ++c) cg[c] = cg[shift + c];
				}
				if (nw > cigar_cap) atomicExch(err_flag, BMH_E_CIGAR_CAP);
			}
		}
		if (live) out[idx].score = score, out[idx].n_cigar = n_cigar;
	}
}

int launch_global_narrow(bmh_ctx *ctx, int wlo, const uint8_t *d_pool, const bmh_glb_task_t *d_tasks, int64_t n, bmh_glb_result_t *d_res,
                         uint32_t *d_cigar, const uint32_t *d_order, const uint32_t *d_count, int rows_cap, const uint8_t *d_band)
{
	if (n <= 0) return BMH_OK;
	if (wlo != 0 && wlo != 4) return BMH_E_ARG;
	const long long grid = std::min<long long>((n + 63) / 64, (long long)ctx->ncu * 4 * (wlo == 0 ? BMH_GN_WAVES_LO : BMH_GN_WAVES_HI));
	int rc = ensure(ctx, ctx->d_zslab, (size_t)grid * (size_t)rows_cap * (size_t)kNarrowBlocks * 64 * 4);
	if (rc) return rc;
	const bool sym = ctx->dev.o_del + ctx->dev.e_del == ctx->dev.o_ins + ctx->dev.e_ins;
#define BMH_LAUNCH_GN(WW, SS)                                                                                                   \
	hipLaunchKernelGGL((global_narrow_kernel<WW, SS>), dim3((unsigned)grid), dim3(64), 0, ctx->stream, d_pool, d_tasks, d_order, d_band, \
	                   d_count, (long long)n, d_res, d_cigar, ctx->dev, (uint32_t *)ctx->d_zslab.p, rows_cap, ctx->d_err)
	if (wlo == 0 && sym) BMH_LAUNCH_GN(0, true);
	else if (wlo == 0) BMH_LAUNCH_GN(0, false);
	else if (sym) BMH_LAUNCH_GN(4, true);
	else BMH_LAUNCH_GN(4, false);
#undef BMH_LAUNCH_GN
	BMH_HIP(ctx, hipGetLastError());
// ... 5 lines not shown
```

### bwa-mem-quickassist_amd/csrc/seedext.hip

```cpp
#include <algorithm>

#include "bmh_ctx.h"
#include "bmh_device.h"

namespace bmh {

struct SeedP {
	int a, w, pen_clip5, pen_clip3, max_mat;
	int limit;
	int qmax;
};

struct SeedState {
	int qb, rbl, truesc, sc0, aw0;
	uint32_t r2;
};

__device__ __forceinline__ uint32_t wave_append(bool pred, uint32_t *counter)
{
	const unsigned long long m = __builtin_amdgcn_ballot_w64(pred);
	if (m == 0) return 0;
	const int leader = __builtin_ctzll(m);
	const int lane = (int)__builtin_amdgcn_mbcnt_hi(~0u, __builtin_amdgcn_mbcnt_lo(~0u, 0u));
	uint32_t base = 0;
	if (lane == leader) base = atomicAdd(counter, (uint32_t)__builtin_popcountll(m));
	base = (uint32_t)__builtin_amdgcn_readlane((int)base, leader);
	return base + (uint32_t)__builtin_popcountll(m & ((1ull << lane) - 1ull));
}

__device__ __forceinline__ void store_task(bmh_ext_task_t *t, uint64_t q_off, uint64_t t_off, int qlen, int tlen, int h0,
                                           int w, int end_bonus, unsigned flags)
{
	uint4 *p = (uint4 *)t;
	p[0] = make_uint4((uint32_t)q_off, (uint32_t)(q_off >> 32), (uint32_t)t_off, (uint32_t)(t_off >> 32));
	p[1] = make_uint4((uint32_t)qlen | (uint32_t)tlen << 16, (uint32_t)h0, (uint32_t)(w & 0xffff) | (uint32_t)end_bonus << 16, flags);
}

constexpr int kMakeThreads = 1024;

struct MakeBin {
	uint32_t *lh;
	__device__ __forceinline__ void begin(const ExtBinned &b)
	{
		if (b.band) return;
		for (int t = threadIdx.x; t < kSortBins * kSortKeysHost; t += kMakeThreads) lh[t] = 0;
		__syncthreads();
	}
	__device__ __forceinline__ void put(const ExtBinned &b, long long i, bool has, int qlen, int tlen, int h0)
	{
		uint16_t bk = kNoTask;
		if (b.band) bk = has ? 0 : kNoTask;
		else if (has) {
			bk = (uint16_t)ext_binkey_of(b.rule, qlen, tlen, h0, (size_t)i);
			atomicAdd(&lh[bk], 1u);
		}
		b.binkey[i] = bk;
	}
	__device__ __forceinline__ void end(const ExtBinned &b)
	{
		if (b.band) return;
		__syncthreads();
		for (int t = threadIdx.x; t < kSortBins * kSortKeysHost; t += kMakeThreads)
			if (lh[t]) atomicAdd(&b.hist[t], lh[t]);
	}
};

__global__ __launch_bounds__(kMakeThreads) void seed_left_make_bin(const bmh_seed_task_t *__restrict__ S, long long n, SeedP sp,
                                                                   bmh_ext_task_t *__restrict__ T, SeedState *__restrict__ ST,
                                                                   ExtBinned bin)
{
	__shared__ uint32_t lh[kSortBins * kSortKeysHost];
	MakeBin mb = {lh};
	mb.begin(bin);
	const long long chunk = (n + gridDim.x - 1) / gridDim.x, lo = chunk * blockIdx.x, hi = min(lo + chunk, n);
	for (long long i = lo + threadIdx.x; i < hi; i += kMakeThreads) {
		const bmh_seed_task_t s = S[i];
		const int rq = s.l_query - s.qbeg - s.len, rt = s.wlen - s.rbeg - s.len;
		bool has = false;
		if (s.qbeg < 0 || s.len <= 0 || rq < 0 || s.rbeg < 0 || rt < 0 || s.qbeg > 65535 || rq > 65535 || s.rbeg > 65535 || rt > 65535 ||
		    (long long)s.l_query * max(sp.max_mat, sp.a) > sp.limit || s.qbeg > sp.qmax || rq > sp.qmax) {
			atomicExch(bin.rule.err_flag, BMH_E_RANGE);
			SeedState st = {0, 0, -1, -1, sp.w, 0xffffffffu};
			ST[i] = st;
		} else if (s.qbeg > 0) {
			const uint64_t tl = (uint64_t)s.rbeg;
			store_task(&T[i], s.q_off + (uint64_t)(s.qbeg - 1), tl > 0 ? s.t_off + tl - 1 : s.t_off, s.qbeg, s.rbeg, s.len * sp.a, sp.w,
			           sp.pen_clip5, BMH_F_QREV | BMH_F_TREV | (s.flags & BMH_F_TPAC));
			SeedState st = {0, 0, -1, -1, sp.w, 0};
			ST[i] = st;
			has = true;
		} else {
			SeedState st = {0, 0, s.len * sp.a, s.len * sp.a, sp.w, 0};
			ST[i] = st;
		}
		mb.put(bin, i, has, s.qbeg, s.rbeg, s.len * sp.a);
	}
	mb.end(bin);
}

template <bool RIGHT>
__global__ __launch_bounds__(256) void seed_try(const bmh_seed_task_t *__restrict__ S, long long n, SeedP sp,
                                                const bmh_ext_task_t *__restrict__ T, const bmh_ext_result_t *__restrict__ X,
                                                bmh_ext_task_t *__restrict__ T2, uint32_t *__restrict__ cnt,
                                                SeedState *__restrict__ ST)
{
	const long long i = (long long)blockIdx.x * 256 + threadIdx.x;
	bool again = false;
	if (i < n && ST[i].r2 != 0xffffffffu) {
		const bmh_seed_task_t s = S[i];
		const bool has = RIGHT ? s.qbeg + s.len != s.l_query : s.qbeg > 0;
		if (has) {
// ... 160 lines not shown
```

### bwa-mem-quickassist_amd/host/glbband_core.h

```cpp
#ifndef BMH_GLBBAND_CORE_H
#define BMH_GLBBAND_CORE_H

#include <stdint.h>

#ifdef __HIPCC__
#define BMH_GB_HD __host__ __device__ __attribute__((always_inline))
#else
#define BMH_GB_HD
#endif

BMH_GB_HD static inline int bmh_gb_code(int b) { return b > 4 ? 4 : b; }

BMH_GB_HD static inline int bmh_glbband_amax(const int8_t *mat)
{
	int k, a = mat[0];
	for (k = 1; k < 25; ++k) a = mat[k] > a ? mat[k] : a;
	return a;
}

BMH_GB_HD static inline uint64_t bmh_gb_ld8(const uint8_t *p)
{
	uint64_t v;
	__builtin_memcpy(&v, p, 8);
	return v;
}

typedef struct {
	const uint8_t *t0, *q0, *t1, *q1;
	int n, two, gap;
} bmh_gb_walk_t;
typedef struct {
	int s1, d, b;
} bmh_gb_part_t;

BMH_GB_HD static inline bmh_gb_walk_t bmh_glbband_walk(int o_del, int e_del, int o_ins, int e_ins, const uint8_t *q, int qlen, const uint8_t *t,
                                                       int tlen)
{
	const int delta = qlen - tlen;
	bmh_gb_walk_t w;
	w.t0 = t, w.q0 = q, w.t1 = delta < 0 ? t - delta : t, w.q1 = delta > 0 ? q + delta : q;
	w.n = delta > 0 ? tlen : qlen, w.two = delta != 0;
	w.gap = delta > 0 ? o_ins + e_ins * delta : delta < 0 ? o_del + e_del * -delta : 0;
	return w;
}

BMH_GB_HD static inline bmh_gb_part_t bmh_glbband_part(const int8_t *mat, const bmh_gb_walk_t *w, int from, int to)
{
	bmh_gb_part_t r;
	int p = from, k, s1 = 0, run = 0, best = 0;
	for (; p + 8 <= to; p += 8) {
		const uint64_t a1 = bmh_gb_ld8(w->t1 + p), b1 = bmh_gb_ld8(w->q1 + p);
		uint64_t a0 = 0, b0 = 0;
		if (w->two) a0 = bmh_gb_ld8(w->t0 + p), b0 = bmh_gb_ld8(w->q0 + p);
		for (k = 0; k < 8; ++k) {
			const int v1 = mat[bmh_gb_code((int)(a1 >> (8 * k) & 255)) * 5 + bmh_gb_code((int)(b1 >> (8 * k) & 255))];
			s1 += v1;
			if (w->two) {
				run += mat[bmh_gb_code((int)(a0 >> (8 * k) & 255)) * 5 + bmh_gb_code((int)(b0 >> (8 * k) & 255))] - v1;
				best = run > best ? run : best;
			}
		}
	}
	for (; p < to; ++p) {
		const int v1 = mat[bmh_gb_code(w->t1[p]) * 5 + bmh_gb_code(w->q1[p])];
		s1 += v1;
		if (w->two) {
			run += mat[bmh_gb_code(w->t0[p]) * 5 + bmh_gb_code(w->q0[p])] - v1;
			best = run > best ? run : best;
		}
	}
	r.s1 = s1, r.d = run, r.b = best;
	return r;
}

BMH_GB_HD static inline void bmh_glbband_join(bmh_gb_part_t *acc, const bmh_gb_part_t *nx)
{
	acc->b = acc->d + nx->b > acc->b ? acc->d + nx->b : acc->b;
	acc->d += nx->d, acc->s1 += nx->s1;
}

BMH_GB_HD static inline int bmh_glbband_lb(const int8_t *mat, int o_del, int e_del, int o_ins, int e_ins, const uint8_t *q, int qlen,
                                           const uint8_t *t, int tlen)
{
	const bmh_gb_walk_t w = bmh_glbband_walk(o_del, e_del, o_ins, e_ins, q, qlen, t, tlen);
	const bmh_gb_part_t r = bmh_glbband_part(mat, &w, 0, w.n);
	return r.s1 + r.b - w.gap;
}

BMH_GB_HD static inline int bmh_glbband_from_lb(int amax, int o_del, int e_del, int o_ins, int e_ins, int qlen, int tlen, int w, int lb)
{
	const int delta = qlen - tlen, ad = delta < 0 ? -delta : delta;
	const long long K = (long long)amax + e_ins + e_del;
	const long long xp = (long long)amax * qlen - o_ins - o_del + (long long)e_del * delta - lb;
	const long long xm = (long long)amax * tlen - o_ins - o_del - (long long)e_ins * delta - lb;
	long long need = ad;
	if (xp >= 0 && xp / K > need) need = xp / K;
	if (xm >= 0 && xm / K > need) need = xm / K;
	return need < w ? (int)need : w;
}

BMH_GB_HD static inline int bmh_glbband_applies(int amax, int o_del, int e_del, int o_ins, int e_ins)
{
	return amax > 0 && o_del >= 0 && e_del >= 0 && o_ins >= 0 && e_ins >= 0;
}

BMH_GB_HD static inline int bmh_glbband_weff(const int8_t *mat, int o_del, int e_del, int o_ins, int e_ins, const uint8_t *q, int qlen,
                                             const uint8_t *t, int tlen, int w)
{
	const int delta = qlen - tlen, ad = delta < 0 ? -delta : delta;
	const int amax = bmh_glbband_amax(mat);
	if (w < ad || qlen < 1 || tlen < 1 || !bmh_glbband_applies(amax, o_del, e_del, o_ins, e_ins)) return w;
	return bmh_glbband_from_lb(amax, o_del, e_del, o_ins, e_ins, qlen, tlen, w,
	                           bmh_glbband_lb(mat, o_del, e_del, o_ins, e_ins, q, qlen, t, tlen));
}

#endif
```

### include/bwamem_hip.h

```cpp
#ifndef BWAMEM_HIP_H
#define BWAMEM_HIP_H

#include <stddef.h>
#include <stdint.h>

#ifdef __cplusplus
extern "C" {
#endif

#define BMH_VERSION 310

enum {
	BMH_OK = 0,
	BMH_E_NODEVICE = -1,
	BMH_E_HIP = -2,
	BMH_E_ARG = -3,
	BMH_E_RANGE = -4,
	BMH_E_NOMEM = -5,
	BMH_E_CIGAR_CAP = -6
};

typedef struct bmh_params {
	int32_t o_del, e_del, o_ins, e_ins;
	int32_t zdrop;
// ... 44 lines not shown
const char *bmh_last_error(const bmh_ctx_t *ctx);

int bmh_device_count(int *n);
int bmh_ctx_create(bmh_ctx_t **ctx, int device);
int bmh_ctx_destroy(bmh_ctx_t *ctx);
int bmh_ctx_set_params(bmh_ctx_t *ctx, const bmh_params_t *p);
int bmh_ctx_set_stream(bmh_ctx_t *ctx, void *hip_stream);
int bmh_ctx_set_pac(bmh_ctx_t *ctx, const uint8_t *pac, int64_t l_pac);
int bmh_ctx_sync(bmh_ctx_t *ctx);
int bmh_ctx_set_wide_extension(bmh_ctx_t *ctx, int enable);
int bmh_ctx_set_wide_sw(bmh_ctx_t *ctx, int enable);
int bmh_ctx_set_qcap(bmh_ctx_t *ctx, int max_qlen);

typedef void (*bmh_gate_fn)(void);
int bmh_set_device_gate(bmh_gate_fn enter, bmh_gate_fn leave);
void bmh_set_wait_mode(int blocking);

int bmh_extend_batch(bmh_ctx_t *ctx, const uint8_t *seqpool, size_t pool_bytes,
                     const bmh_ext_task_t *tasks, int64_t n, bmh_ext_result_t *results);
int bmh_global_batch(bmh_ctx_t *ctx, const uint8_t *seqpool, size_t pool_bytes,
                     const bmh_glb_task_t *tasks, int64_t n, bmh_glb_result_t *results,
                     uint32_t *cigar_pool, size_t cigar_pool_words);

int bmh_upload_pool(bmh_ctx_t *ctx, const uint8_t *seqpool, size_t pool_bytes);

int bmh_extend_batch_device(bmh_ctx_t *ctx, const uint8_t *d_seqpool,
                            const bmh_ext_task_t *d_tasks, int64_t n,
                            bmh_ext_result_t *d_results, const uint32_t *d_order);
int bmh_global_batch_device(bmh_ctx_t *ctx, const uint8_t *d_seqpool,
                            const bmh_glb_task_t *d_tasks, int64_t n,
                            bmh_glb_result_t *d_results, uint32_t *d_cigar_pool,
                            const uint32_t *d_order);

int bmh_extend_batch_sharded(bmh_ctx_t *const *ctxs, int n_ctx, const uint8_t *seqpool,
                             size_t pool_bytes, const bmh_ext_task_t *tasks, int64_t n,
                             bmh_ext_result_t *results);
struct bmh_seed_task; struct bmh_seed_result; struct bmh_sw_task; struct bmh_sw_result;
int bmh_seedext_batch_sharded(bmh_ctx_t *const *ctxs, int n_ctx, const uint8_t *seqpool, size_t pool_bytes,
                              const struct bmh_seed_task *tasks, int64_t n, struct bmh_seed_result *results);
int bmh_global_batch_sharded(bmh_ctx_t *const *ctxs, int n_ctx, const uint8_t *seqpool, size_t pool_bytes,
                             const bmh_glb_task_t *tasks, int64_t n, bmh_glb_result_t *results,
                             uint32_t *cigar_pool, size_t cigar_pool_words);
int bmh_sw_batch_sharded(bmh_ctx_t *const *ctxs, int n_ctx, const uint8_t *seqpool, size_t pool_bytes,
                         const struct bmh_sw_task *tasks, int64_t n, struct bmh_sw_result *results);

typedef struct bmh_seed_task {
	uint64_t q_off;
	uint64_t t_off;
	int32_t l_query;
	int32_t qbeg, len;
	int32_t rbeg;
	int32_t wlen;
	uint16_t flags;
	uint16_t rsv_;
} bmh_seed_task_t;

typedef struct bmh_seed_result {
	int32_t qb, qe;
	int32_t rb, re;
	int32_t score, truesc;
	int32_t w;
	int32_t n_ext;
} bmh_seed_result_t;

int bmh_seedext_batch(bmh_ctx_t *ctx, const uint8_t *seqpool, size_t pool_bytes, const bmh_seed_task_t *tasks, int64_t n,
                      bmh_seed_result_t *results);
int bmh_seedext_batch_device(bmh_ctx_t *ctx, const uint8_t *d_seqpool, const bmh_seed_task_t *d_tasks, int64_t n,
                             bmh_seed_result_t *d_results);
int bmh_seedext_submit(bmh_ctx_t *ctx, const bmh_seed_task_t *tasks, int64_t n);
int bmh_seedext_wait(bmh_ctx_t *ctx, bmh_seed_result_t *results);
typedef struct bmh_seedext_stats {
	int64_t seeds, left_tasks, left_retries, right_tasks, right_retries;
} bmh_seedext_stats_t;
int bmh_seedext_stats(const bmh_ctx_t *ctx, bmh_seedext_stats_t *st);

int bmh_last_kernel_ms(bmh_ctx_t *ctx, float *ms);
int bmh_set_kernel_timing(bmh_ctx_t *ctx, int enable);
int bmh_last_extend_bin_ms(bmh_ctx_t *ctx, float ms[6]);
int bmh_extend_bin_ms_sum(bmh_ctx_t *ctx, double ms[6], long long *launches, int reset);
int bmh_extend_wide_stats(const bmh_ctx_t *ctx, int64_t *tasks, float *ms);
int bmh_last_global_bin_ms(bmh_ctx_t *ctx, float ms[3]);
int bmh_last_global_bands(bmh_ctx_t *ctx, uint8_t *bands, int64_t n);
int bmh_last_global_bin_counts(bmh_ctx_t *ctx, uint32_t counts[8]);
int bmh_ctx_set_extend_rows(bmh_ctx_t *ctx, int64_t cap);
int bmh_last_extend_rows(bmh_ctx_t *ctx, uint16_t *rows, int64_t n);
int bmh_last_extend_bands(bmh_ctx_t *ctx, uint8_t *bands, int64_t n);
int bmh_global_long_stats(const bmh_ctx_t *ctx, int64_t *tasks, float *ms);
int bmh_sw_wide_stats(const bmh_ctx_t *ctx, int64_t *tasks, float *ms);
int bmh_last_seedext_round_ms(bmh_ctx_t *ctx, float ms[4]);

typedef struct bmh_seed {
	int64_t rbeg;
	int32_t qbeg, len;
} bmh_seed_t;

typedef struct bmh_chain {
	int32_t n, m;
	int64_t pos;
	bmh_seed_t *seeds;
} bmh_chain_t;

typedef struct bmh_chain_v {
	size_t n, m;
	bmh_chain_t *a;
} bmh_chain_v;

typedef struct bmh_alnreg {
	int64_t rb, re;
	int32_t qb, qe;
	int32_t score, truesc, sub, csub, sub_n, w, seedcov, secondary;
	uint64_t hash;
} bmh_alnreg_t;

typedef struct bmh_alnreg_v {
	size_t n, m;
	bmh_alnreg_t *a;
} bmh_alnreg_v;

typedef struct bmh_read {
	int32_t l_seq;
	const uint8_t *seq;
} bmh_read_t;

typedef int (*bmh_chain_pre_fn)(void *user, int read, int chain, bmh_alnreg_v *av);

int bmh_chain2aln_batch(bmh_ctx_t *ctx, int64_t l_pac, const uint8_t *pac, int n_reads,
                        const bmh_read_t *reads, const bmh_chain_v *chains, bmh_chain_pre_fn pre,
                        void *pre_user, bmh_alnreg_v *regs);

int bmh_chains2regs_batch(bmh_ctx_t *ctx, int64_t l_pac, const uint8_t *pac, int n_reads, const bmh_read_t *reads,
                          const bmh_chain_v *chains, int min_seed_len, bmh_alnreg_v *regs);

typedef struct bmh_cigar_req {
	int32_t read;
	int32_t qb, qe;
	int64_t rb, re;
	int32_t truesc;
	int32_t reg_w;
} bmh_cigar_req_t;

typedef struct bmh_cigar_res {
	int32_t score;
	int32_t n_cigar;
	int32_t NM;
	int32_t tries;
	uint32_t cigar_off;
	uint32_t md_off;
	uint32_t md_len;
	uint32_t rsv_;
} bmh_cigar_res_t;

int bmh_reg2cigar_batch(bmh_ctx_t *ctx, int64_t l_pac, const uint8_t *pac, const bmh_read_t *reads, int64_t n_req,
                        const bmh_cigar_req_t *reqs, bmh_cigar_res_t *results, uint32_t *cigar_pool,
                        size_t cigar_words, char *md_pool, size_t md_bytes);

#define BMH_REGION_CIGAR_CUT 1u
#define BMH_REGION_MD_CUT 2u
typedef struct bmh_region_req {
	uint64_t q_src;
	int64_t rb;
	uint64_t o_off;
	int32_t ql, tl;
	int32_t truesc;
	int32_t task[3];
} bmh_region_req_t;
typedef struct bmh_region_res {
// ... 297 lines not shown
```

Before: 209.5 million reads/s.

## Add speculative narrow-band pre-pass for wide global alignments and diagonal fast path

Adds an opt-in (BMH_GLB_TRY) speculative pass that runs wide-band global tasks first in the 32-column lane kernel with band 15. Tasks whose score certifies that the narrow band is exact are kept, and the rest are appended to redo lists for the wide kernels, so the wider DP cost is only paid where needed. Separately, the narrow kernel gets a default-on shortcut: w==0, equal-length tasks emit a single M CIGAR op instead of running traceback. The try pass adds an extra launch, atomics and scratch buffers, and it is off by default.

```diff
diff --git a/bwa-mem-quickassist_amd/__init__.py b/bwa-mem-quickassist_amd/__init__.py
--- a/bwa-mem-quickassist_amd/__init__.py
+++ b/bwa-mem-quickassist_amd/__init__.py
@@ -190,6 +190,7 @@
         L.bmh_last_global_bin_ms.argtypes = [C.c_void_p, C.POINTER(C.c_float)]
         L.bmh_last_global_bands.argtypes = [C.c_void_p, C.c_void_p, C.c_int64]
         L.bmh_last_global_bin_counts.argtypes = [C.c_void_p, C.c_void_p]
+        L.bmh_last_global_try_counts.argtypes = [C.c_void_p, C.c_void_p]
         L.bmh_ctx_set_extend_rows.argtypes = [C.c_void_p, C.c_int64]
         L.bmh_last_extend_rows.argtypes = [C.c_void_p, C.c_void_p, C.c_int64]
         L.bmh_last_extend_bands.argtypes = [C.c_void_p, C.c_void_p, C.c_int64]
@@ -405,6 +406,11 @@
         self._check(lib().bmh_last_global_bin_counts(self._h, _ptr(counts)))
         return counts
 
+    def last_global_try_counts(self):
+        counts = np.zeros(5, dtype=np.uint32)
+        self._check(lib().bmh_last_global_try_counts(self._h, _ptr(counts)))
+        return counts
+
     def set_extend_rows(self, cap):
         self._check(lib().bmh_ctx_set_extend_rows(self._h, int(cap)))
 
diff --git a/bwa-mem-quickassist_amd/csrc/api.hip b/bwa-mem-quickassist_amd/csrc/api.hip
--- a/bwa-mem-quickassist_amd/csrc/api.hip
+++ b/bwa-mem-quickassist_amd/csrc/api.hip
@@ -284,6 +284,7 @@
 	if (const char *m = getenv("BMH_GLB_C32")) ctx->glb_c32 = atoi(m) != 0;
 	if (const char *m = getenv("BMH_GLB_NARROW")) ctx->glb_narrow = atoi(m) != 0;
 	if (const char *m = getenv("BMH_GLB_EXACT")) ctx->glb_exact = atoi(m) >= 7 ? 7 : atoi(m) >= 3 ? 3 : 0;
+	if (const char *m = getenv("BMH_GLB_TRY")) ctx->glb_try = atoi(m) != 0;
 	if (const char *m = getenv("BMH_GRID_MULT")) ctx->grid_mult = atoi(m) > 0 ? atoi(m) : 1;
 	if (const char *m = getenv("BMH_EXT_SCHED")) ctx->ext_sched = atoi(m) >= 0 && atoi(m) <= 4 ? atoi(m) : -1;
 	*out = ctx;
@@ -299,7 +300,7 @@
 	(void)hipSetDevice(ctx->device);
 	if (ctx->stream) (void)stream_wait(ctx, ctx->stream);
 	free_buf(ctx->d_pool), free_buf(ctx->d_tasks), free_buf(ctx->d_res), free_buf(ctx->d_order);
-	free_buf(ctx->d_cigar), free_buf(ctx->d_scratch), free_buf(ctx->d_bins), free_buf(ctx->d_gband), free_buf(ctx->d_ext_rows), free_buf(ctx->d_eband), free_buf(ctx->d_zslab), free_buf(ctx->d_sw), free_buf(ctx->d_swrm);
+	free_buf(ctx->d_cigar), free_buf(ctx->d_scratch), free_buf(ctx->d_bins), free_buf(ctx->d_gband), free_buf(ctx->d_gredo), free_buf(ctx->d_ext_rows), free_buf(ctx->d_eband), free_buf(ctx->d_zslab), free_buf(ctx->d_sw), free_buf(ctx->d_swrm);
 	free_buf(ctx->d_seedws), free_buf(ctx->d_region), free_buf(ctx->d_chain), free_buf(ctx->d_wide_slab), free_buf(ctx->d_c2r);
 	if (ctx->d_wide_stat) (void)hipFree(ctx->d_wide_stat);
 	if (ctx->d_swl_stat) (void)hipFree(ctx->d_swl_stat);
@@ -616,6 +617,20 @@
 	BMH_HIP(ctx, hipSetDevice(ctx->device));
 	BMH_HIP(ctx, stream_wait(ctx, ctx->stream));
 	BMH_HIP(ctx, hipMemcpy(counts, ctx->d_bins.p, kSortBins * sizeof(uint32_t), hipMemcpyDeviceToHost));
+	return BMH_OK;
+}
+
+int bmh_last_global_try_counts(bmh_ctx_t *ctx, uint32_t counts[5])
+{
+	if (!ctx || !counts) return BMH_E_ARG;
+	for (int k = 0; k < 5; ++k) counts[k] = 0;
+	if (!ctx->glb_try || ctx->glb_mode != 0) return BMH_OK;
+	if (!ctx->gtry_valid || !ctx->d_gredo.p) return BMH_E_ARG;
+	uint32_t h[5];
+	BMH_HIP(ctx, hipSetDevice(ctx->device));
+	BMH_HIP(ctx, stream_wait(ctx, ctx->stream));
+	BMH_HIP(ctx, hipMemcpy(h, ctx->d_gredo.p, sizeof h, hipMemcpyDeviceToHost));
+	counts[0] = h[3], counts[1] = h[4], counts[2] = h[0], counts[3] = h[1], counts[4] = h[2];
 	return BMH_OK;
 }
 
@@ -1400,6 +1415,8 @@
 	BMH_HIP(ctx, hipSetDevice(ctx->device));
 	if (ctx->glb_narrow && (1 + (size_t)kSortBins) * N + 16 > ctx->d_gband.cap) ctx->gband_n = 0;
 	if ((16 + (size_t)kSortBins * kSortKeysHost + (N + 1) / 2 + 1 + (size_t)kSortBins * N) * 4 > ctx->d_bins.cap) ctx->gbins_valid = false;
+	if (ctx->glb_try && ctx->glb_mode == 0 && 64 + 3 * N * 4 + 3 * N + 16 > ctx->d_gredo.cap) ctx->gtry_valid = false;
+	if (ctx->glb_try && ctx->glb_mode == 0 && (rc = ensure(ctx, ctx->d_gredo, 64 + 3 * N * 4 + 3 * N + 16))) return rc;
 	if ((rc = ensure(ctx, ctx->d_pool, pool_bytes + 16)) || (rc = ensure(ctx, ctx->d_tasks, N * 40 + 64)) || (rc = ensure(ctx, ctx->d_res, N * 32 + 64)) ||
 	    (rc = ensure(ctx, ctx->d_cigar, (cigar_words + 4) * 4)) ||
 	    (rc = ensure(ctx, ctx->d_bins, (16 + (size_t)kSortBins * kSortKeysHost + (N + 1) / 2 + 1 + (size_t)kSortBins * N) * 4)) ||
diff --git a/bwa-mem-quickassist_amd/csrc/bmh_ctx.h b/bwa-mem-quickassist_amd/csrc/bmh_ctx.h
--- a/bwa-mem-quickassist_amd/csrc/bmh_ctx.h
+++ b/bwa-mem-quickassist_amd/csrc/bmh_ctx.h
@@ -36,6 +36,9 @@
 	int glb_narrow = 1;
 	int glb_c32 = 1;
 	int glb_exact = 7;
+	int glb_try = 0;
+	DevBuf d_gredo;
+	bool gtry_valid = false;
 	bool gbins_valid = false;
 	DevBuf d_gband;
 	int64_t gband_n = 0;
@@ -263,9 +266,16 @@
 int sort_tasks_begin(bmh_ctx *ctx, int64_t n, uint32_t **counts, uint32_t **lists);
 int sort_tasks_finish(bmh_ctx *ctx, int64_t n, const uint32_t *d_order, unsigned blocks, const uint32_t *d_n = nullptr,
                       uint32_t *d_total = nullptr, const uint8_t *d_payload = nullptr, uint8_t *d_plists = nullptr);
+constexpr int kGlbTryBand = 15;
+struct GlbTry {
+	uint32_t *order;
+	uint8_t *band;
+	uint32_t *count;
+	uint32_t *stat;
+};
 int launch_global_lane(bmh_ctx *ctx, int c, const uint8_t *d_pool, const bmh_glb_task_t *d_tasks, int64_t n,
                        bmh_glb_result_t *d_res, uint32_t *d_cigar, const uint32_t *d_order, const uint32_t *d_count,
-                       int rows_cap, const uint8_t *d_band = nullptr);
+                       int rows_cap, const uint8_t *d_band = nullptr, const GlbTry *tr = nullptr);
 int launch_global_narrow(bmh_ctx *ctx, int wlo, const uint8_t *d_pool, const bmh_glb_task_t *d_tasks, int64_t n, bmh_glb_result_t *d_res,
                          uint32_t *d_cigar, const uint32_t *d_order, const uint32_t *d_count, int rows_cap, const uint8_t *d_band = nullptr);
 constexpr int kExtBins = 6;
diff --git a/bwa-mem-quickassist_amd/csrc/bmh_device.h b/bwa-mem-quickassist_amd/csrc/bmh_device.h
--- a/bwa-mem-quickassist_amd/csrc/bmh_device.h
+++ b/bwa-mem-quickassist_amd/csrc/bmh_device.h
@@ -53,6 +53,18 @@
 }
 
 __device__ __forceinline__ int uni(int v) { return __builtin_amdgcn_readfirstlane(v); }
+
+__device__ __forceinline__ uint32_t wave_append(bool pred, uint32_t *counter)
+{
+	const unsigned long long m = __builtin_amdgcn_ballot_w64(pred);
+	if (m == 0) return 0;
+	const int leader = __builtin_ctzll(m);
+	const int lane = (int)__builtin_amdgcn_mbcnt_hi(~0u, __builtin_amdgcn_mbcnt_lo(~0u, 0u));
+	uint32_t base = 0;
+	if (lane == leader) base = atomicAdd(counter, (uint32_t)__builtin_popcountll(m));
+	base = (uint32_t)__builtin_amdgcn_readlane((int)base, leader);
+	return base + (uint32_t)__builtin_popcountll(m & ((1ull << lane) - 1ull));
+}
 
 __device__ __forceinline__ int mat_at(const DevParams &P, int idx)
 {
diff --git a/bwa-mem-quickassist_amd/csrc/global_kernel.hip b/bwa-mem-quickassist_amd/csrc/global_kernel.hip
--- a/bwa-mem-quickassist_amd/csrc/global_kernel.hip
+++ b/bwa-mem-quickassist_amd/csrc/global_kernel.hip
@@ -293,7 +293,7 @@
                   bmh_glb_result_t *d_res, uint32_t *d_cigar, const uint32_t *d_order, int qmax, int tmax,
                   int wmax, int wgate, const GlbLongShape *lg)
 {
-	ctx->gband_n = 0, ctx->gbins_valid = false;
+	ctx->gband_n = 0, ctx->gbins_valid = false, ctx->gtry_valid = false;
 	if (n <= 0) return BMH_OK;
 	int rc;
 	const size_t N = (size_t)n;
@@ -350,6 +350,24 @@
 	                   binkey, ctx->dev, lane_ok ? 1 : 0, rows_cap, longb ? kGlbLdsQcap : 65535, band, ctx->glb_c32, ctx->glb_exact);
 	if ((rc = sort_tasks_finish(ctx, n, d_order, (unsigned)cg, nullptr, nullptr, band, blists))) return rc;
 	ctx->gbins_valid = true;
+	uint32_t *tstat = nullptr;
+	if (lane_ok && ctx->glb_try) {
+		if ((rc = ensure(ctx, ctx->d_gredo, 64 + 3 * N * 4 + 3 * N + 16))) return rc;
+		tstat = (uint32_t *)ctx->d_gredo.p;
+		BMH_HIP(ctx, hipMemsetAsync(tstat, 0, 64, ctx->stream));
+		ctx->gtry_valid = true;
+	}
+	auto wide = [&](int c, int b, int r) -> int {
+		const uint32_t *lst = lists + (size_t)b * N, *cnt = counts + b;
+		const uint8_t *bl = blists ? blists + (size_t)b * N : nullptr;
+		if (tstat && wgate > kGlbTryBand) {
+			const GlbTry tr = {tstat + 16 + (size_t)r * N, blists ? (uint8_t *)(tstat + 16 + 3 * N) + (size_t)r * N : nullptr, tstat + r, tstat + 3};
+			int rc2 = launch_global_lane(ctx, 32, d_pool, d_tasks, n, d_res, d_cigar, lst, cnt, rows_cap, bl, &tr);
+			if (rc2) return rc2;
+			lst = tr.order, cnt = tr.count, bl = tr.band;
+		}
+		return launch_global_lane(ctx, c, d_pool, d_tasks, n, d_res, d_cigar, lst, cnt, rows_cap, bl);
+	};
 	const bool tm = ctx->timing;
 	if (tm) BMH_HIP(ctx, hipEventRecord(ctx->ev0, ctx->stream));
 	if (lane_ok) {
@@ -361,14 +379,10 @@
 		if (ctx->glb_c32 && (rc = launch_global_lane(ctx, 32, d_pool, d_tasks, n, d_res, d_cigar, lists + 5 * N, counts + 5, rows_cap,
 		                                             blists ? blists + 5 * N : nullptr)))
 			return rc;
-		if ((rc = launch_global_lane(ctx, 64, d_pool, d_tasks, n, d_res, d_cigar, lists, counts + 0, rows_cap, blists))) return rc;
+		if ((rc = wide(64, 0, 0))) return rc;
 		if (tm) BMH_HIP(ctx, hipEventRecord(ctx->ev_gbin[1], ctx->stream));
-		if (wgate > 31 && (rc = launch_global_lane(ctx, 96, d_pool, d_tasks, n, d_res, d_cigar, lists + 3 * N, counts + 3, rows_cap,
-		                                             blists ? blists + 3 * N : nullptr)))
-			return rc;
-		if (wgate > 47 && (rc = launch_global_lane(ctx, 128, d_pool, d_tasks, n, d_res, d_cigar, lists + N, counts + 1, rows_cap,
-		                                             blists ? blists + N : nullptr)))
-			return rc;
+		if (wgate > 31 && (rc = wide(96, 3, 2))) return rc;
+		if (wgate > 47 && (rc = wide(128, 1, 1))) return rc;
 	}
 	if (tm) BMH_HIP(ctx, hipEventRecord(ctx->ev_gbin[2], ctx->stream));
 	{
diff --git a/bwa-mem-quickassist_amd/csrc/global_lane.hip b/bwa-mem-quickassist_amd/csrc/global_lane.hip
--- a/bwa-mem-quickassist_amd/csrc/global_lane.hip
+++ b/bwa-mem-quickassist_amd/csrc/global_lane.hip
@@ -5,6 +5,7 @@
 #include "bmh_ctx.h"
 #include "bmh_device.h"
 #include "seq_stream.h"
+#include "../host/glbband_core.h"
 
 namespace bmh {
 
@@ -30,12 +31,13 @@
 #endif
 
 
-template <int C, bool FAST, bool SYM>
+template <int C, bool FAST, bool SYM, bool TRY = false>
 __global__ __launch_bounds__(64, (C <= 32 ? BMH_GL_WAVES32 : C <= 64 ? BMH_GL_WAVES64 : C <= 96 ? BMH_GL_WAVES96 : BMH_GL_WAVES128)) void global_lane_kernel(
     const uint8_t *__restrict__ pool, const bmh_glb_task_t *__restrict__ tasks, const uint32_t *__restrict__ order,
     const uint8_t *__restrict__ band, const uint32_t *__restrict__ count, long long n, bmh_glb_result_t *__restrict__ out,
-    uint32_t *__restrict__ cigar_pool, DevParams P, uint32_t *__restrict__ zslab, int rows_cap, int *__restrict__ err_flag)
+    uint32_t *__restrict__ cigar_pool, DevParams P, uint32_t *__restrict__ zslab, int rows_cap, int *__restrict__ err_flag, GlbTry tr)
 {
+	static_assert(!TRY || 2 * kGlbTryBand + 2 <= C, "the try band fits the slots");
 	constexpr int NW = (C + 31) / 32, NQ = C / 4, NB = C / 8;
 	__shared__ uint2 srow[8];
 	extern __shared__ __attribute__((aligned(16))) uint8_t dyn_lds[];
@@ -58,14 +60,16 @@
 		const uint4 ta = tp[0], tb = tp[1];
 		const uint64_t q_off = (uint64_t)ta.y << 32 | ta.x;
 		const int qlen = (int)(tb.x & 0xffff), tlen = (int)(tb.x >> 16);
-		const int w = band ? (int)band[pos] : (int)tb.y;
+		const int wown = band ? (int)band[pos] : (int)tb.y;
+		const int w = TRY ? kGlbTryBand : wown;
 		const bool want = (int)tb.w > 0;
-		const bool bad = w < 0 || 2 * w + 2 > C || tlen > rows_cap;
+		const bool bad = !TRY && (w < 0 || 2 * w + 2 > C || tlen > rows_cap);
 		if (valid && bad) {
 			out[idx].score = INT32_MIN, out[idx].n_cigar = 0;
 			atomicExch(err_flag, BMH_E_RANGE);
 		}
-		const bool live = valid && !bad;
+		bool live = valid && !bad;
+		if (TRY) live = live && tlen <= rows_cap && bmh_glbband_tried(P.max_mat, P.o_del, e_del, P.o_ins, e_ins, qlen, tlen, wown, kGlbTryBand);
 
 		int R[C + 1], QW[NQ];
 #pragma unroll
@@ -202,6 +206,24 @@
 		if (tlen == 0) score = qlen == 0 ? 0 : (qlen <= w ? -(P.o_ins + e_ins * qlen) : kNeg16);
 		if (score <= -kGlbLaneWorst) score = -0x40000000;
 
+		if (TRY) {
+			int lane_now;
+			asm volatile("v_mbcnt_lo_u32_b32 %0, -1, 0\n\tv_mbcnt_hi_u32_b32 %0, -1, %0" : "=v"(lane_now));
+			const bool valid2 = base + lane_now < cnt;
+			const long long pos2 = cnt - 1 - (valid2 ? base + lane_now : base);
+			const int wown2 = band ? (int)band[pos2] : ((const int *)(tasks + idx))[5];
+			const bool cert = live && bmh_glbband_certified(P.max_mat, P.o_del, e_del, P.o_ins, e_ins, qlen, tlen, wown2, kGlbTryBand, score);
+			const bool redo = valid2 && !cert;
+			const uint32_t at = wave_append(redo, tr.count);
+			if (redo) {
+				tr.order[at] = idx;
+				if (tr.band) tr.band[at] = (uint8_t)wown2;
+			}
+			const int ntried = __builtin_popcountll(__builtin_amdgcn_ballot_w64(live)), ncert = __builtin_popcountll(__builtin_amdgcn_ballot_w64(cert));
+			if (lane_now == 0 && ntried) atomicAdd(tr.stat, (uint32_t)ntried), atomicAdd(tr.stat + 1, (uint32_t)ncert);
+			live = cert;
+		}
+
 		const uint2 tc = *(const uint2 *)((const uint8_t *)(tasks + idx) + 24);
 		const uint32_t cigar_off = tc.x;
 		const int cigar_cap = (int)tc.y;
@@ -279,9 +301,11 @@
 
 int launch_global_lane(bmh_ctx *ctx, int c, const uint8_t *d_pool, const bmh_glb_task_t *d_tasks, int64_t n,
                        bmh_glb_result_t *d_res, uint32_t *d_cigar, const uint32_t *d_order, const uint32_t *d_count,
-                       int rows_cap, const uint8_t *d_band)
+                       int rows_cap, const uint8_t *d_band, const GlbTry *tr)
 {
 	if (n <= 0) return BMH_OK;
+	if (tr && c != 32) return BMH_E_ARG;
+	const GlbTry tv = tr ? *tr : GlbTry{nullptr, nullptr, nullptr, nullptr};
 	int ncu = 256;
 	(void)hipDeviceGetAttribute(&ncu, hipDeviceAttributeMultiprocessorCount, ctx->device);
 	long long grid = (n + 63) / 64;
@@ -293,9 +317,10 @@
 	const bool fast = ctx->glb_fast != 0;
 	const bool sym = ctx->dev.o_del + ctx->dev.e_del == ctx->dev.o_ins + ctx->dev.e_ins;
 	const size_t lds = (size_t)std::max(c, kStreamRows) * 64;
-#define BMH_LAUNCH_GL2(CC, FF, SS)                                                                                             \
-	hipLaunchKernelGGL((global_lane_kernel<CC, FF, SS>), dim3((unsigned)grid), dim3(64), lds, ctx->stream, d_pool, d_tasks, d_order, \
-	                   d_band, d_count, (long long)n, d_res, d_cigar, ctx->dev, (uint32_t *)ctx->d_zslab.p, rows_cap, ctx->d_err)
+#define BMH_LAUNCH_GL3(CC, FF, SS, TT)                                                                                         \
+	hipLaunchKernelGGL((global_lane_kernel<CC, FF, SS, TT>), dim3((unsigned)grid), dim3(64), lds, ctx->stream, d_pool, d_tasks, d_order, \
+	                   d_band, d_count, (long long)n, d_res, d_cigar, ctx->dev, (uint32_t *)ctx->d_zslab.p, rows_cap, ctx->d_err, tv)
+#define BMH_LAUNCH_GL2(CC, FF, SS) BMH_LAUNCH_GL3(CC, FF, SS, false)
 #define BMH_LAUNCH_GL(CC)                                                                                                      \
 	do {                                                                                                                       \
 		if (fast && sym) BMH_LAUNCH_GL2(CC, true, true);                                                                       \
@@ -303,13 +328,19 @@
 		else if (sym) BMH_LAUNCH_GL2(CC, false, true);                                                                         \
 		else BMH_LAUNCH_GL2(CC, false, false);                                                                                 \
 	} while (0)
-	if (c == 32) BMH_LAUNCH_GL(32);
+	if (tr) {
+		if (fast && sym) BMH_LAUNCH_GL3(32, true, true, true);
+		else if (fast) BMH_LAUNCH_GL3(32, true, false, true);
+		else if (sym) BMH_LAUNCH_GL3(32, false, true, true);
+		else BMH_LAUNCH_GL3(32, false, false, true);
+	} else if (c == 32) BMH_LAUNCH_GL(32);
 	else if (c == 64) BMH_LAUNCH_GL(64);
 	else if (c == 96) BMH_LAUNCH_GL(96);
 	else if (c == 128) BMH_LAUNCH_GL(128);
 	else return BMH_E_ARG;
 #undef BMH_LAUNCH_GL
 #undef BMH_LAUNCH_GL2
+#undef BMH_LAUNCH_GL3
 	BMH_HIP(ctx, hipGetLastError());
 	return BMH_OK;
 }
diff --git a/bwa-mem-quickassist_amd/csrc/global_narrow.hip b/bwa-mem-quickassist_amd/csrc/global_narrow.hip
--- a/bwa-mem-quickassist_amd/csrc/global_narrow.hip
+++ b/bwa-mem-quickassist_amd/csrc/global_narrow.hip
@@ -141,6 +141,10 @@
 #define BMH_GN_WAVES_HI 6
 #endif
 
+#ifndef BMH_GN_DIAG0
+#define BMH_GN_DIAG0 1
+#endif
+
 template <int WLO, bool SYM>
 __global__ __launch_bounds__(64, (WLO == 0 ? BMH_GN_WAVES_LO : BMH_GN_WAVES_HI)) void global_narrow_kernel(
     const uint8_t *__restrict__ pool, const bmh_glb_task_t *__restrict__ tasks, const uint32_t *__restrict__ order,
@@ -173,6 +177,7 @@
 			atomicExch(err_flag, BMH_E_RANGE);
 		}
 		const bool live = valid && !bad;
+		const bool diag = BMH_GN_DIAG0 && WLO == 0 && w == 0 && qlen == tlen && qlen >= 1 && want;
 
 		int score = kNeg16;
 		for (unsigned long long todo = __builtin_amdgcn_ballot_w64(live); todo != 0;) {
@@ -181,7 +186,7 @@
 			int sc = kNeg16;
 #define BMH_GN_CASE(WW)                                                                                                \
 	case WW:                                                                                                           \
-		sc = narrow_rows<WW, SYM>(mine, want, qlen, tlen, idx, pool, tasks, P, srow, lds, zbase, rows_cap);            \
+		sc = narrow_rows<WW, SYM>(mine, want && !diag, qlen, tlen, idx, pool, tasks, P, srow, lds, zbase, rows_cap);            \
 		break;
 			switch (wc) {
 				BMH_GN_CASE(WLO)
@@ -200,11 +205,12 @@
 		const uint32_t cigar_off = tc.x;
 		const int cigar_cap = (int)tc.y;
 		int n_cigar = 0;
-		if (__builtin_amdgcn_ballot_w64(live && want)) {
+		if (live && diag) cigar_pool[cigar_off] = (uint32_t)qlen << 4, n_cigar = 1;
+		if (__builtin_amdgcn_ballot_w64(live && want && !diag)) {
 			__builtin_amdgcn_fence(__ATOMIC_SEQ_CST, "workgroup");
 			uint32_t *cg = cigar_pool + cigar_off;
 			int ti = tlen - 1, tk = min(qlen, tlen - 1 + w + 1) - 1, which = 0, last_op = 0, last_len = 0, nw = 0;
-			const bool on = live && want;
+			const bool on = live && want && !diag;
 			uint32_t *strip = (uint32_t *)lds;
 			int cblk = -1, ctop = -1;
 			while (__builtin_amdgcn_ballot_w64(on && ti >= 0 && tk >= 0)) {
diff --git a/bwa-mem-quickassist_amd/csrc/seedext.hip b/bwa-mem-quickassist_amd/csrc/seedext.hip
--- a/bwa-mem-quickassist_amd/csrc/seedext.hip
+++ b/bwa-mem-quickassist_amd/csrc/seedext.hip
@@ -15,18 +15,6 @@
 	int qb, rbl, truesc, sc0, aw0;
 	uint32_t r2;
 };
-
-__device__ __forceinline__ uint32_t wave_append(bool pred, uint32_t *counter)
-{
-	const unsigned long long m = __builtin_amdgcn_ballot_w64(pred);
-	if (m == 0) return 0;
-	const int leader = __builtin_ctzll(m);
-	const int lane = (int)__builtin_amdgcn_mbcnt_hi(~0u, __builtin_amdgcn_mbcnt_lo(~0u, 0u));
-	uint32_t base = 0;
-	if (lane == leader) base = atomicAdd(counter, (uint32_t)__builtin_popcountll(m));
-	base = (uint32_t)__builtin_amdgcn_readlane((int)base, leader);
-	return base + (uint32_t)__builtin_popcountll(m & ((1ull << lane) - 1ull));
-}
 
 __device__ __forceinline__ void store_task(bmh_ext_task_t *t, uint64_t q_off, uint64_t t_off, int qlen, int tlen, int h0,
                                            int w, int end_bonus, unsigned flags)
diff --git a/bwa-mem-quickassist_amd/host/glbband_core.h b/bwa-mem-quickassist_amd/host/glbband_core.h
--- a/bwa-mem-quickassist_amd/host/glbband_core.h
+++ b/bwa-mem-quickassist_amd/host/glbband_core.h
@@ -104,6 +104,17 @@
 	return amax > 0 && o_del >= 0 && e_del >= 0 && o_ins >= 0 && e_ins >= 0;
 }
 
+BMH_GB_HD static inline int bmh_glbband_tried(int amax, int o_del, int e_del, int o_ins, int e_ins, int qlen, int tlen, int w, int wtry)
+{
+	const int delta = qlen - tlen, ad = delta < 0 ? -delta : delta;
+	return bmh_glbband_applies(amax, o_del, e_del, o_ins, e_ins) && qlen >= 1 && tlen >= 1 && ad <= wtry && w > wtry;
+}
+
+BMH_GB_HD static inline int bmh_glbband_certified(int amax, int o_del, int e_del, int o_ins, int e_ins, int qlen, int tlen, int w, int wtry, int score)
+{
+	return bmh_glbband_from_lb(amax, o_del, e_del, o_ins, e_ins, qlen, tlen, w, score) <= wtry;
+}
+
 BMH_GB_HD static inline int bmh_glbband_weff(const int8_t *mat, int o_del, int e_del, int o_ins, int e_ins, const uint8_t *q, int qlen,
                                              const uint8_t *t, int tlen, int w)
 {
diff --git a/include/bwamem_hip.h b/include/bwamem_hip.h
--- a/include/bwamem_hip.h
+++ b/include/bwamem_hip.h
@@ -150,6 +150,7 @@
 int bmh_last_global_bin_ms(bmh_ctx_t *ctx, float ms[3]);
 int bmh_last_global_bands(bmh_ctx_t *ctx, uint8_t *bands, int64_t n);
 int bmh_last_global_bin_counts(bmh_ctx_t *ctx, uint32_t counts[8]);
+int bmh_last_global_try_counts(bmh_ctx_t *ctx, uint32_t counts[5]);
 int bmh_ctx_set_extend_rows(bmh_ctx_t *ctx, int64_t cap);
 int bmh_last_extend_rows(bmh_ctx_t *ctx, uint16_t *rows, int64_t n);
 int bmh_last_extend_bands(bmh_ctx_t *ctx, uint8_t *bands, int64_t n);
```

Result: no change. 211.2 million reads/s (median of 6 runs) (+0.8%).
